# edogariu/artist-style-transfer

Hardware: NVIDIA B200
Metric: train_images_per_sec_256 (higher is better)
Workload: dtype bf16

## Files before the change

artist_style_transfer_b200/csrc/conv_hx.cu:

```cuda
#include "px_common.cuh"

namespace ast {

constexpr int HX_EPI_WARPS = 8;
constexpr int HX_WPROD_WARP = 2 + HX_EPI_WARPS;
constexpr int HX_THREADS = 32 * (HX_WPROD_WARP + 1);
constexpr int HX_MAX_PBUF = 4;
constexpr int HX_MAX_WBUF = 4;
constexpr int HX_TW = 8;

struct HxParams {
  int mi, mj, tiles_i, tiles_j, n_img, n_slices, R;
  int ntaps, kchunks, kc, cout, flags;
  int nblk, cb, sy, soy, sox, cstat;
  int oy[4], ox[4];
  int dy_min, dx_min, ph, pw;
  int patch_bytes, patch_tx, n_pbuf, n_wbuf, tg, ngroups;
  unsigned idesc;
  long long total_tiles;
  short tdy[AST_MAX_TAPS];
  short tdx[AST_MAX_TAPS];
};

__device__ __forceinline__ void hx_tile(const HxParams& p, long long tile, int& slice, int& tj, int& ti, int& img) {
  long long r = tile;
  slice = (int)(r % p.n_slices); r /= p.n_slices;
  tj = (int)(r % p.tiles_j); r /= p.tiles_j;
  ti = (int)(r % p.tiles_i);
  img = (int)(r / p.tiles_i);
}

template <int KIND>
__global__ void __launch_bounds__(HX_THREADS, 1)
conv_hx_kernel(const __grid_constant__ CUtensorMap tm_in, const __grid_constant__ CUtensorMap tm_w, const HxParams p,
               const float* __restrict__ bias, const Img32 add, const Img32 mask, const Img32 out,
               double* __restrict__ stats) {
  extern __shared__ unsigned char smem_raw[];
  __shared__ __align__(8) unsigned long long pfull[HX_MAX_PBUF], pempty[HX_MAX_PBUF], wfull[HX_MAX_WBUF], wempty[HX_MAX_WBUF];
  __shared__ __align__(8) unsigned long long tfull_bar[2], tempty_bar[2];
  __shared__ unsigned tmem_slot;
  __shared__ unsigned s_tapoff[AST_MAX_TAPS];

  unsigned char* smem_p = (unsigned char*)(((uintptr_t)smem_raw + 1023) & ~(uintptr_t)1023);
  unsigned char* smem_w = smem_p + (size_t)p.n_pbuf * p.patch_bytes;
  const int warp = threadIdx.x >> 5, lane = threadIdx.x & 31;
  constexpr int W_TILE = 128 * 128;
  const int w_slot = p.tg * W_TILE;

  if (threadIdx.x == 0) {
    asm volatile("prefetch.tensormap [%0];" ::"l"(&tm_in) : "memory");
    asm volatile("prefetch.tensormap [%0];" ::"l"(&tm_w) : "memory");
    for (int s = 0; s < p.n_pbuf; ++s) { mbar_init(&pfull[s], 1); mbar_init(&pempty[s], 1); }
    for (int s = 0; s < p.n_wbuf; ++s) { mbar_init(&wfull[s], 1); mbar_init(&wempty[s], 1); }
    for (int a = 0; a < 2; ++a) { mbar_init(&tfull_bar[a], 1); mbar_init(&tempty_bar[a], 32 * HX_EPI_WARPS); }
    asm volatile("fence.mbarrier_init.release.cluster;" ::: "memory");
    asm volatile("fence.proxy.async.shared::cta;" ::: "memory");
  }
  if (threadIdx.x >= 64 && threadIdx.x - 64 < p.ntaps) {
    const int t = threadIdx.x - 64;
    s_tapoff[t] = (unsigned)((p.tdy[t] * p.pw + p.tdx[t]) * 128) >> 4;
  }
  if (warp == 1) {
    asm volatile("tcgen05.alloc.cta_group::1.sync.aligned.shared::cta.b32 [%0], %1;" ::"r"(smem_u32(&tmem_slot)), "r"(512u) : "memory");
    asm volatile("tcgen05.relinquish_alloc_permit.cta_group::1.sync.aligned;" ::: "memory");
  }
  tc_fence_before();
  __syncthreads();
  tc_fence_after();
  const unsigned tmem_base = tmem_slot;

  if (warp == 0) {
    if (lane == 0) {
      int s = 0; unsigned ph = 0;
      for (long long tile = blockIdx.x; tile < p.total_tiles; tile += gridDim.x) {
        int slice, tj, ti, img;
        hx_tile(p, tile, slice, tj, ti, img);
        const int x0 = tj * HX_TW + p.dx_min, y0 = ti * p.R * p.sy + p.dy_min;
        for (int kc = 0; kc < p.kchunks; ++kc) {
          mbar_wait(&pempty[s], ph ^ 1);
          mbar_expect_tx(&pfull[s], (unsigned)p.patch_tx);
          tma_load_4d(smem_p + (size_t)s * p.patch_bytes, &tm_in, &pfull[s], kc * p.kc, x0, y0, img);
          if (++s == p.n_pbuf) { s = 0; ph ^= 1; }
        }
      }
    }
  } else if (warp == HX_WPROD_WARP) {
    if (lane == 0) {
      int s = 0; unsigned ph = 0;
      for (long long tile = blockIdx.x; tile < p.total_tiles; tile += gridDim.x) {
        int slice, tj, ti, img;
        hx_tile(p, tile, slice, tj, ti, img);
        for (int kc = 0; kc < p.kchunks; ++kc) {
          for (int gidx = 0; gidx < p.ngroups; ++gidx) {
            mbar_wait(&wempty[s], ph ^ 1);
            mbar_expect_tx(&wfull[s], (unsigned)w_slot);
            tma_load_3d(smem_w + (size_t)s * w_slot, &tm_w, &wfull[s], kc * p.kc, slice * 128, gidx * p.tg);
            if (++s == p.n_wbuf) { s = 0; ph ^= 1; }
          }
        }
      }
    }
  } else if (warp == 1) {
    int ps = 0; unsigned pph = 0; int ws = 0; unsigned wph = 0; int as = 0; unsigned aph = 0;
    const unsigned hi_w = ((8u * 128u) >> 4) | (1u << 14) | (2u << 29);
    const unsigned hi_p = (((unsigned)(p.sy * p.pw) * 128u) >> 4) | (1u << 14) | (2u << 29);
    const unsigned w_base = smem_u32(smem_w), p_base = smem_u32(smem_p);
    for (long long tile = blockIdx.x; tile < p.total_tiles; tile += gridDim.x) {
      mbar_wait(&tempty_bar[as], aph ^ 1);
      tc_fence_after();
      const unsigned d_tmem = tmem_base + (unsigned)(as * 256);
      for (int kc = 0; kc < p.kchunks; ++kc) {
        mbar_wait(&pfull[ps], pph);
        const unsigned p_lo = (((p_base + (unsigned)ps * (unsigned)p.patch_bytes) & 0x3FFFFu) >> 4) | (1u << 16);
        for (int gidx = 0; gidx < p.ngroups; ++gidx) {
          mbar_wait(&wfull[ws], wph);
          tc_fence_after();
          if (lane == 0) {
            const unsigned w_lo = (((w_base + (unsigned)ws * (unsigned)w_slot) & 0x3FFFFu) >> 4) | (1u << 16);
            const int t0 = gidx * p.tg, t1 = min(p.ntaps, t0 + p.tg);
            for (int t = t0; t < t1; ++t) {
              const unsigned a_lo = w_lo + (unsigned)(t - t0) * (W_TILE >> 4);
              const unsigned b_lo = p_lo + s_tapoff[t];
              tc_mma<KIND>(d_tmem, pack_desc64(a_lo, hi_w), pack_desc64(b_lo, hi_p), p.idesc, (kc | t) ? 1u : 0u);
              tc_mma<KIND>(d_tmem, pack_desc64(a_lo + 2, hi_w), pack_desc64(b_lo + 2, hi_p), p.idesc, 1u);
              tc_mma<KIND>(d_tmem, pack_desc64(a_lo + 4, hi_w), pack_desc64(b_lo + 4, hi_p), p.idesc, 1u);
              tc_mma<KIND>(d_tmem, pack_desc64(a_lo + 6, hi_w), pack_desc64(b_lo + 6, hi_p), p.idesc, 1u);
            }
            tc_commit(&wempty[ws]);
            if (gidx == p.ngroups - 1) {
              tc_commit(&pempty[ps]);
              if (kc == p.kchunks - 1) tc_commit(&tfull_bar[as]);
            }
          }
          __syncwarp();
          if (++ws == p.n_wbuf) { ws = 0; wph ^= 1; }
        }
        if (++ps == p.n_pbuf) { ps = 0; pph ^= 1; }
      }
      if (++as == 2) { as = 0; aph ^= 1; }
    }
  } else if (warp < HX_WPROD_WARP) {
    const int q = warp & 3;
    const int par = (warp - 2) >> 2;
    const int L = q * 32 + lane;
    const int blk = L / p.cb, chl = L % p.cb;
    const int oy_g = p.oy[blk], ox_g = p.ox[blk];
    PxStep st;
    st.out_r = p.soy * out.sh; st.out_c = p.sox * out.sw;
    st.add_r = p.soy * add.sh; st.add_c = p.sox * add.sw;
    st.mask_r = p.soy * mask.sh; st.mask_c = p.sox * mask.sw;
    const int jlim = min(p.mj, ox_g < out.w ? (out.w - ox_g + p.sox - 1) / p.sox : 0);
    const int ilim = min(p.mi, oy_g < out.h ? (out.h - oy_g + p.soy - 1) / p.soy : 0);
    int as = 0; unsigned aph = 0;
    double s1 = 0.0, s2 = 0.0;
    int s_img = -1, s_ch = 0;
    for (long long tile = blockIdx.x; tile < p.total_tiles; tile += gridDim.x) {
      int slice, tj, ti, img;
      hx_tile(p, tile, slice, tj, ti, img);
      const int ch = slice * 128 + chl;
      if (stats && (img != s_img || ch != s_ch)) {
        if (s_img >= 0) { double* srow = stats + ((long long)s_img * p.cstat + s_ch) * 2; atomicAdd(srow, s1); atomicAdd(srow + 1, s2); }
        s1 = s2 = 0.0; s_img = img; s_ch = ch;
      }
      const float b = bias ? bias[ch] : 0.f;
      mbar_wait(&tfull_bar[as], aph);
      tc_fence_after();
      const unsigned taddr0 = tmem_base + ((unsigned)(q * 32) << 16) + (unsigned)(as * 256);
      const int j0 = tj * HX_TW;
      const int nvc = max(0, min(HX_TW, jlim - j0));
#pragma unroll 1
      for (int c0 = par * 32; c0 < 256; c0 += 8 * HX_EPI_WARPS) {
        const int r0 = c0 >> 3;
        if (r0 >= p.R) break;
        float v[32];
        tc_ld32(taddr0 + c0, v);
        const int i0 = ti * p.R + r0;
        const int nvr = max(0, min(min(4, p.R - r0), ilim - i0));
        const int oy = oy_g + p.soy * i0, ox = ox_g + p.sox * j0;
        PxOff off;
        off.out = img * out.sn + oy * out.sh + ox * out.sw;
        off.add = add.ptr ? img * add.sn + oy * add.sh + ox * add.sw : 0;
        off.mask = mask.ptr ? img * mask.sn + oy * mask.sh + ox * mask.sw : 0;
        if (nvr == 4 && nvc == 8)
          px_chunk<8, true>(v, off, st, 4, 8, ch, lane, b, p.flags, add, mask, out, stats != nullptr, s1, s2);
        else if (nvr > 0 && nvc > 0)
          px_chunk<8>(v, off, st, nvr, nvc, ch, lane, b, p.flags, add, mask, out, stats != nullptr, s1, s2);
      }
      tc_fence_before();
      mbar_arrive(&tempty_bar[as]);
      if (++as == 2) { as = 0; aph ^= 1; }
    }
    if (stats && s_img >= 0) { double* srow = stats + ((long long)s_img * p.cstat + s_ch) * 2; atomicAdd(srow, s1); atomicAdd(srow + 1, s2); }
  }

  tc_fence_before();
  __syncthreads();
  if (warp == 1) {
    tc_fence_after();
    asm volatile("tcgen05.dealloc.cta_group::1.sync.aligned.b32 %0, %1;" ::"r"(tmem_base), "r"(512u) : "memory");
  }
}

struct HxGeom {
  int mi, mj, ntaps, flags;
  int nblk, cb, sy, soy, sox, cstat;
  int oy[4], ox[4];
  const int16_t* dy;
  const int16_t* dx;
  double* stats;
};

static int hx_launch(const ast_image* in, const void* weights, const float* bias, const ast_image* add, const ast_image* mask,
                     const ast_image* out, const HxGeom& g, int cout, cudaStream_t stream) {
  if (!img32_ok(out) || !img32_ok(add) || !img32_ok(mask)) return 0;
  const int esz = in->dtype == AST_F32 ? 4 : 2;
  if ((in->c * esz) % 128 != 0 || cout % 128 != 0) return 0;
  int dy_min = 1 << 30, dy_max = -(1 << 30), dx_min = 1 << 30, dx_max = -(1 << 30);
  for (int t = 0; t < g.ntaps; ++t) {
    dy_min = g.dy[t] < dy_min ? g.dy[t] : dy_min; dy_max = g.dy[t] > dy_max ? g.dy[t] : dy_max;
    dx_min = g.dx[t] < dx_min ? g.dx[t] : dx_min; dx_max = g.dx[t] > dx_max ? g.dx[t] : dx_max;
  }
  if (dx_max - dx_min > 4 || dy_max - dy_min > 8) return 0;
  HxParams p;
  memset(&p, 0, sizeof(p));
  p.kc = 128 / esz;
  p.kchunks = in->c / p.kc;
  if (g.ntaps * p.kchunks < 8) return 0;
  EncodeTiledFn encode = get_encode();
  if (!encode) return 0;
  p.mi = g.mi; p.mj = g.mj;
  p.nblk = g.nblk; p.cb = g.cb; p.sy = g.sy; p.soy = g.soy; p.sox = g.sox;
  for (int b = 0; b < 4; ++b) { p.oy[b] = g.oy[b]; p.ox[b] = g.ox[b]; }
  p.cstat = g.nblk == 1 ? cout : g.cb;
  p.ntaps = g.ntaps; p.flags = g.flags; p.cout = cout; p.n_img = in->n; p.n_slices = cout / 128;
  p.dy_min = dy_min; p.dx_min = dx_min;
  for (int t = 0; t < g.ntaps; ++t) { p.tdy[t] = g.dy[t] - dy_min; p.tdx[t] = g.dx[t] - dx_min; }
  p.pw = HX_TW + (dx_max - dx_min);
  const int budget = 225 * 1024 - 1024;
  p.tg = g.ntaps % 3 == 0 ? 3 : (g.ntaps % 2 == 0 ? 2 : (g.ntaps >= 3 ? 3 : g.ntaps));
  p.ngroups = (g.ntaps + p.tg - 1) / p.tg;
  const int w_slot = p.tg * 128 * 128;
  auto patch_rows = [&](int R) { return (R - 1) * p.sy + (dy_max - dy_min) + 1; };
  int rmax = 32;
  while (rmax > 2 && (2 * ((p.pw * patch_rows(rmax) * 128 + 1023) & ~1023) + 2 * w_slot > budget || patch_rows(rmax) > 256)) rmax -= 2;
  p.tiles_i = (p.mi + rmax - 1) / rmax;
  p.R = (p.mi + p.tiles_i - 1) / p.tiles_i;
  p.R = (p.R + 1) & ~1;
  p.tiles_i = (p.mi + p.R - 1) / p.R;
  p.tiles_j = (p.mj + HX_TW - 1) / HX_TW;
  p.total_tiles = (long long)p.n_img * p.tiles_i * p.tiles_j * p.n_slices;
  p.ph = patch_rows(p.R);
  p.patch_tx = p.pw * p.ph * 128;
  p.patch_bytes = (p.patch_tx + 1023) & ~1023;
  p.n_pbuf = 2;
  p.n_wbuf = (budget - p.n_pbuf * p.patch_bytes) / w_slot;
  if (p.n_wbuf < 2) return 0;
  if (p.n_wbuf > HX_MAX_WBUF) p.n_wbuf = HX_MAX_WBUF;
  if (budget - p.n_pbuf * p.patch_bytes - p.n_wbuf * w_slot >= p.patch_bytes) p.n_pbuf = 3;
  const unsigned fmt = tc_operand_fmt(in->dtype);
  p.idesc = (1u << 4) | (fmt << 7) | (fmt << 10) | ((unsigned)((8 * p.R) >> 3) << 17) | ((128u >> 4) << 24);

  alignas(64) CUtensorMap tm_in, tm_w;
  const CUtensorMapDataType dt = tc_tmap_dtype(in->dtype);
  {
    cuuint64_t dims[4] = {(cuuint64_t)in->c, (cuuint64_t)in->w, (cuuint64_t)in->h, (cuuint64_t)in->n};
    cuuint64_t strides[3] = {(cuuint64_t)in->sw * esz, (cuuint64_t)in->sh * esz, (cuuint64_t)in->sn * esz};
    cuuint32_t box[4] = {(cuuint32_t)p.kc, (cuuint32_t)p.pw, (cuuint32_t)p.ph, 1};
    cuuint32_t estr[4] = {1, 1, 1, 1};
    if (int r = cached_tensor_map(encode, &tm_in, dt, 4, in->ptr, dims, strides, box, estr, CU_TENSOR_MAP_SWIZZLE_128B,
                                  CU_TENSOR_MAP_L2_PROMOTION_L2_128B)) return r;
  }
  {
    cuuint64_t dims[3] = {(cuuint64_t)in->c, (cuuint64_t)cout, (cuuint64_t)g.ntaps};
    cuuint64_t strides[2] = {(cuuint64_t)in->c * esz, (cuuint64_t)cout * in->c * esz};
    cuuint32_t box[3] = {(cuuint32_t)p.kc, 128, (cuuint32_t)p.tg};
    cuuint32_t estr[3] = {1, 1, 1};
    if (int r = cached_tensor_map(encode, &tm_w, dt, 3, const_cast<void*>(weights), dims, strides, box, estr,
                                  CU_TENSOR_MAP_SWIZZLE_128B, CU_TENSOR_MAP_L2_PROMOTION_L2_256B)) return r;
  }
  const size_t smem = 1024 + (size_t)p.n_pbuf * p.patch_bytes + (size_t)p.n_wbuf * w_slot;
  const int grid = (int)(p.total_tiles < num_sms() ? p.total_tiles : num_sms());
  cudaError_t e;
  if (in->dtype != AST_F32) {
    e = set_max_smem(conv_hx_kernel<0>, smem);
    if (e == cudaSuccess) launch_k(conv_hx_kernel<0>, grid, HX_THREADS, smem, stream, tm_in, tm_w, p, bias, to_img32(add), to_img32(mask), to_img32(out), g.stats);
  } else {
    e = set_max_smem(conv_hx_kernel<1>, smem);
    if (e == cudaSuccess) launch_k(conv_hx_kernel<1>, grid, HX_THREADS, smem, stream, tm_in, tm_w, p, bias, to_img32(add), to_img32(mask), to_img32(out), g.stats);
  }
  if (e != cudaSuccess) { set_error("conv_hx: cudaFuncSetAttribute failed: %s", cudaGetErrorString(e)); return (int)e; }
  count_launch();
  return 1;
}

int conv_gather_hx(const ast_image* in, const void* weights, const float* bias, const ast_image* add,
                   const ast_image* mask, const ast_image* out, const ast_gather_geom* g, int cpad, bool thin,
                   cudaStream_t stream) {
  static const int enabled = [] { const char* e = getenv("AST_CONV_HX"); return e ? atoi(e) : 1; }();
  if (!enabled) return 0;
  if (thin || g->pooled || g->w_img_stride != 0 || g->si != 1 || cpad % 128 != 0 || out->c != cpad) return 0;
  int dy_min = 1 << 30, dy_max = -(1 << 30);
  for (int t = 0; t < g->ntaps; ++t) { dy_min = g->dy[t] < dy_min ? g->dy[t] : dy_min; dy_max = g->dy[t] > dy_max ? g->dy[t] : dy_max; }
  if (dy_max - dy_min > 4) return 0;
  HxGeom hg;
  memset(&hg, 0, sizeof(hg));
  hg.mi = g->mi; hg.mj = g->mj; hg.ntaps = g->ntaps; hg.flags = g->flags;
  hg.nblk = 1; hg.cb = 128; hg.sy = 1; hg.soy = hg.sox = g->so;
  hg.oy[0] = g->oy0; hg.ox[0] = g->ox0;
  hg.dy = g->dy; hg.dx = g->dx; hg.stats = g->stats;
  const int r = hx_launch(in, weights, bias, add, mask, out, hg, cpad, stream);
  if (r != 1) return r;
  count_work(FAM_CONV_HX, conv_flops(in, out, g), conv_bytes(in, out, g, add, mask));
  AST_CUDA_LAUNCH_CHECK();
  return 1;
}

int conv_stacked_hx(const ast_image* in, const void* weights, const float* bias, const ast_image* add,
                    const ast_image* mask, const ast_image* out, const ast_stacked_geom* g, cudaStream_t stream) {
  HxGeom hg;
  memset(&hg, 0, sizeof(hg));
  hg.mi = g->mi; hg.mj = g->mj; hg.ntaps = g->nvt; hg.flags = g->flags;
  hg.nblk = g->nblk; hg.cb = 128 / g->nblk; hg.sy = g->sy; hg.soy = g->soy; hg.sox = g->sox;
  for (int b = 0; b < g->nblk; ++b) { hg.oy[b] = g->oy[b]; hg.ox[b] = g->ox[b]; }
  hg.dy = g->dy; hg.dx = g->dx; hg.stats = g->stats;
  return hx_launch(in, weights, bias, add, mask, out, hg, 128, stream);
}

}
```

artist_style_transfer_b200/csrc/conv_px.cu:

```cuda
#include "px_common.cuh"

namespace ast {

constexpr int PX_THREADS = 320;
constexpr int PX_MAX_STAGES = 8;
constexpr int PX_PRODUCERS = 4;

struct PxParams {
  int mi, mj, tw, th, tiles_i, tiles_j, n_img;
  int ntaps, kchunks, kc;
  int si, so, oy0, ox0;
  int cout, flags;
  int w_rows_per_img;
  int stages, w_bytes, a_bytes, stage_bytes, rowb;
  int pairs_per_img;
  unsigned idesc, layout_type, sbo;
  long long total_pairs;
  short dy[AST_MAX_TAPS];
  short dx[AST_MAX_TAPS];
};

template <int KIND>
__global__ void __launch_bounds__(PX_THREADS, 1)
conv_px_kernel(const __grid_constant__ CUtensorMap tm_in, const __grid_constant__ CUtensorMap tm_w, const PxParams p,
               const float* __restrict__ bias, const Img32 add, const Img32 mask, const Img32 out,
               double* __restrict__ stats) {
  extern __shared__ unsigned char smem_raw[];
  __shared__ __align__(8) unsigned long long full_bar[PX_MAX_STAGES], empty_bar[PX_MAX_STAGES], tfull_bar[2], tempty_bar[2];
  __shared__ unsigned tmem_slot;
  unsigned char* smem = (unsigned char*)(((uintptr_t)smem_raw + 1023) & ~(uintptr_t)1023);
  const int warp = threadIdx.x >> 5, lane = threadIdx.x & 31;
  const int ksteps = p.ntaps * p.kchunks;

  if (threadIdx.x == 0) {
    asm volatile("prefetch.tensormap [%0];" ::"l"(&tm_in) : "memory");
    asm volatile("prefetch.tensormap [%0];" ::"l"(&tm_w) : "memory");
    for (int s = 0; s < p.stages; ++s) { mbar_init(&full_bar[s], 1); mbar_init(&empty_bar[s], 1); }
    for (int a = 0; a < 2; ++a) { mbar_init(&tfull_bar[a], 1); mbar_init(&tempty_bar[a], 256); }
    asm volatile("fence.mbarrier_init.release.cluster;" ::: "memory");
    asm volatile("fence.proxy.async.shared::cta;" ::: "memory");
  }
  if (warp == 1) {
    asm volatile("tcgen05.alloc.cta_group::1.sync.aligned.shared::cta.b32 [%0], %1;" ::"r"(smem_u32(&tmem_slot)), "r"(512u) : "memory");
    asm volatile("tcgen05.relinquish_alloc_permit.cta_group::1.sync.aligned;" ::: "memory");
  }
  tc_fence_before();
  __syncthreads();
  tc_fence_after();
  const unsigned tmem_base = tmem_slot;

  if (warp == 0) {
    const int nprod = p.stages < PX_PRODUCERS ? p.stages : PX_PRODUCERS;
    if (lane < nprod) {
      int s = 0, turn = 0; unsigned ph = 0;
      for (long long pair = blockIdx.x; pair < p.total_pairs; pair += gridDim.x) {
        const int img = (int)(pair / p.pairs_per_img);
        const int sp0 = 2 * (int)(pair % p.pairs_per_img);
        const int ti0 = sp0 / p.tiles_j, tj0 = sp0 - ti0 * p.tiles_j;
        const int ti1 = (sp0 + 1) / p.tiles_j, tj1 = (sp0 + 1) - ti1 * p.tiles_j;
        const int x0 = p.si * tj0 * p.tw, y0 = p.si * ti0 * p.th, x1 = p.si * tj1 * p.tw, y1 = p.si * ti1 * p.th;
        const int wrow0 = img * p.w_rows_per_img;
        for (int t = 0; t < p.ntaps; ++t) {
          for (int kc = 0; kc < p.kchunks; ++kc) {
            if (turn == lane) {
              mbar_wait(&empty_bar[s], ph ^ 1);
              unsigned char* sw = smem + (size_t)s * p.stage_bytes;
              mbar_expect_tx(&full_bar[s], (unsigned)p.stage_bytes);
              tma_load_2d(sw, &tm_w, &full_bar[s], kc * p.kc, wrow0 + t * p.cout);
              tma_load_4d(sw + p.w_bytes, &tm_in, &full_bar[s], kc * p.kc, x0 + p.dx[t], y0 + p.dy[t], img);
              tma_load_4d(sw + p.w_bytes + p.a_bytes, &tm_in, &full_bar[s], kc * p.kc, x1 + p.dx[t], y1 + p.dy[t], img);
            }
            if (++turn == nprod) turn = 0;
            if (++s == p.stages) { s = 0; ph ^= 1; }
          }
        }
      }
    }
  } else if (warp == 1) {
    int s = 0; unsigned ph = 0; int as = 0; unsigned aph = 0;
    const int kmma = p.rowb / 32;
    const unsigned desc_hi = (p.sbo >> 4) | (1u << 14) | (p.layout_type << 29);
    for (long long pair = blockIdx.x; pair < p.total_pairs; pair += gridDim.x) {
      mbar_wait(&tempty_bar[as], aph ^ 1);
      tc_fence_after();
      const unsigned d_tmem = tmem_base + (unsigned)(as * 256);
      for (int ks = 0; ks < ksteps; ++ks) {
        mbar_wait(&full_bar[s], ph);
        tc_fence_after();
        if (lane == 0) {
          const unsigned w_addr = smem_u32(smem + (size_t)s * p.stage_bytes);
          const unsigned a_lo = ((w_addr & 0x3FFFFu) >> 4) | (1u << 16);
          const unsigned b_lo = (((w_addr + p.w_bytes) & 0x3FFFFu) >> 4) | (1u << 16);
          tc_mma<KIND>(d_tmem, pack_desc64(a_lo, desc_hi), pack_desc64(b_lo, desc_hi), p.idesc, ks > 0 ? 1u : 0u);
          tc_mma<KIND>(d_tmem, pack_desc64(a_lo + 2, desc_hi), pack_desc64(b_lo + 2, desc_hi), p.idesc, 1u);
          if (kmma == 4) {
            tc_mma<KIND>(d_tmem, pack_desc64(a_lo + 4, desc_hi), pack_desc64(b_lo + 4, desc_hi), p.idesc, 1u);
            tc_mma<KIND>(d_tmem, pack_desc64(a_lo + 6, desc_hi), pack_desc64(b_lo + 6, desc_hi), p.idesc, 1u);
          }
          tc_commit(&empty_bar[s]);
          if (ks == ksteps - 1) tc_commit(&tfull_bar[as]);
        }
        __syncwarp();
        if (++s == p.stages) { s = 0; ph ^= 1; }
      }
      if (++as == 2) { as = 0; aph ^= 1; }
    }
  } else {
    const int q = warp & 3;
    const int half = (warp - 2) >> 2;
    const int ch = q * 32 + lane;
    const bool ch_ok = ch < p.cout;
    const float b = (bias && ch_ok) ? bias[ch] : 0.f;
    int as = 0; unsigned aph = 0;
    double s1 = 0.0, s2 = 0.0;
    int s_img = -1;
    for (long long pair = blockIdx.x; pair < p.total_pairs; pair += gridDim.x) {
      const int img = (int)(pair / p.pairs_per_img);
      if (stats && img != s_img) {
        if (s_img >= 0 && ch_ok) { double* srow = stats + ((long long)s_img * p.cout + ch) * 2; atomicAdd(srow, s1); atomicAdd(srow + 1, s2); }
        s1 = s2 = 0.0; s_img = img;
      }
      const int sp = 2 * (int)(pair % p.pairs_per_img) + half;
      const int ti = sp / p.tiles_j, tj = sp - ti * p.tiles_j;
      mbar_wait(&tfull_bar[as], aph);
      tc_fence_after();
      const unsigned taddr0 = tmem_base + ((unsigned)(q * 32) << 16) + (unsigned)(as * 256 + half * 128);
      if (q * 32 < p.cout) {
        const bool fast = (p.tw & 31) == 0;
        for (int c0 = 0; c0 < 128; c0 += 32) {
          float v[32];
          tc_ld32(taddr0 + c0, v);
          if (fast) {
            const int ty = c0 / p.tw, tx0 = c0 - ty * p.tw;
            const int i = ti * p.th + ty, j0 = tj * p.tw + tx0;
            const int oy = p.oy0 + p.so * i, ox = p.ox0 + p.so * j0;
            int nvalid = 0;
            if (i < p.mi && oy < out.h) {
              const int jlim = min(p.mj, (out.w - p.ox0 + p.so - 1) / p.so);
              nvalid = max(0, min(32, jlim - j0));
            }
            PxOff off;
            off.out = img * out.sn + oy * out.sh + ox * out.sw;
            off.add = add.ptr ? img * add.sn + oy * add.sh + ox * add.sw : 0;
            off.mask = mask.ptr ? img * mask.sn + oy * mask.sh + ox * mask.sw : 0;
            PxStep st;
            st.out_r = st.add_r = st.mask_r = 0;
            st.out_c = p.so * out.sw; st.add_c = p.so * add.sw; st.mask_c = p.so * mask.sw;
            if (nvalid > 0) px_chunk<32>(v, off, st, 1, nvalid, ch, lane, b, p.flags, add, mask, out, stats != nullptr, s1, s2);
          } else {
            const int row = c0 + lane;
            const int ty = row / p.tw, tx = row - ty * p.tw;
            const int i = ti * p.th + ty, j = tj * p.tw + tx;
            const int oy = p.oy0 + p.so * i, ox = p.ox0 + p.so * j;
            const bool valid = i < p.mi && j < p.mj && oy < out.h && ox < out.w;
            PxOff off;
            off.out = valid ? img * out.sn + oy * out.sh + ox * out.sw : -1;
            off.add = add.ptr ? img * add.sn + oy * add.sh + ox * add.sw : 0;
            off.mask = mask.ptr ? img * mask.sn + oy * mask.sh + ox * mask.sw : 0;
            PxStep st = {0, 0, 0, 0, 0, 0};
            px_chunk<0>(v, off, st, 0, 0, ch, lane, b, p.flags, add, mask, out, stats != nullptr, s1, s2);
          }
        }
      }
      tc_fence_before();
      mbar_arrive(&tempty_bar[as]);
      if (++as == 2) { as = 0; aph ^= 1; }
    }
    if (stats && s_img >= 0 && ch_ok) { double* srow = stats + ((long long)s_img * p.cout + ch) * 2; atomicAdd(srow, s1); atomicAdd(srow + 1, s2); }
  }

  tc_fence_before();
  __syncthreads();
  if (warp == 1) {
    tc_fence_after();
    asm volatile("tcgen05.dealloc.cta_group::1.sync.aligned.b32 %0, %1;" ::"r"(tmem_base), "r"(512u) : "memory");
  }
}

int conv_gather_px(const ast_image* in, const void* weights, const float* bias, const ast_image* add,
                   const ast_image* mask, const ast_image* out, const ast_gather_geom* g, int cpad, bool thin,
                   cudaStream_t stream) {
  if (thin || g->pooled || (cpad != 64 && cpad != 128) || out->c != cpad) return 0;
  if (!img32_ok(out) || !img32_ok(add) || !img32_ok(mask)) return 0;
  if (in->dtype == AST_F16) return 0;
  const int esz = in->dtype == AST_F32 ? 4 : 2;
  EncodeTiledFn encode = get_encode();
  if (!encode) return 0;

  PxParams p;
  memset(&p, 0, sizeof(p));
  p.mi = g->mi; p.mj = g->mj; p.si = g->si; p.so = g->so; p.oy0 = g->oy0; p.ox0 = g->ox0;
  p.ntaps = g->ntaps; p.flags = g->flags; p.cout = cpad; p.n_img = in->n;
  for (int t = 0; t < g->ntaps; ++t) { p.dy[t] = g->dy[t]; p.dx[t] = g->dx[t]; }
  pick_tile(p.mi, p.mj, 128, &p.tw, &p.th);
  p.tiles_i = (p.mi + p.th - 1) / p.th;
  p.tiles_j = (p.mj + p.tw - 1) / p.tw;
  p.rowb = (in->c * esz) % 128 == 0 ? 128 : 64;
  p.kc = p.rowb / esz;
  p.kchunks = in->c / p.kc;
  if (p.ntaps * p.kchunks * (p.rowb / 32) < 16) return 0;
  p.w_rows_per_img = 0;
  if (g->w_img_stride) {
    if (g->w_img_stride != (int64_t)g->ntaps * cpad * in->c) return 0;
    p.w_rows_per_img = g->ntaps * cpad;
  }
  p.w_bytes = 128 * p.rowb;
  p.a_bytes = 128 * p.rowb;
  p.stage_bytes = p.w_bytes + 2 * p.a_bytes;
  p.stages = (200 * 1024) / p.stage_bytes;
  if (p.stages > PX_MAX_STAGES) p.stages = PX_MAX_STAGES;
  p.layout_type = p.rowb == 128 ? 2u : 4u;
  p.sbo = 8u * p.rowb;
  const unsigned fmt = tc_operand_fmt(in->dtype);
  p.idesc = (1u << 4) | (fmt << 7) | (fmt << 10) | ((256u >> 3) << 17) | ((128u >> 4) << 24);
  p.pairs_per_img = (p.tiles_i * p.tiles_j + 1) / 2;
  p.total_pairs = (long long)p.n_img * p.pairs_per_img;

  alignas(64) CUtensorMap tm_in, tm_w;
  const CUtensorMapDataType dt = tc_tmap_dtype(in->dtype);
  const CUtensorMapSwizzle sw = p.rowb == 128 ? CU_TENSOR_MAP_SWIZZLE_128B : CU_TENSOR_MAP_SWIZZLE_64B;
  {
    cuuint64_t dims[4] = {(cuuint64_t)in->c, (cuuint64_t)in->w, (cuuint64_t)in->h, (cuuint64_t)in->n};
    cuuint64_t strides[3] = {(cuuint64_t)in->sw * esz, (cuuint64_t)in->sh * esz, (cuuint64_t)in->sn * esz};
    cuuint32_t box[4] = {(cuuint32_t)p.kc, (cuuint32_t)(p.tw * p.si), (cuuint32_t)(p.th * p.si), 1};
    cuuint32_t estr[4] = {1, (cuuint32_t)p.si, (cuuint32_t)p.si, 1};
    if (int r = cached_tensor_map(encode, &tm_in, dt, 4, in->ptr, dims, strides, box, estr, sw, CU_TENSOR_MAP_L2_PROMOTION_L2_128B)) return r;
  }
  {
    const long long rows = (long long)g->ntaps * cpad * (g->w_img_stride ? in->n : 1);
    cuuint64_t dims[2] = {(cuuint64_t)in->c, (cuuint64_t)rows};
    cuuint64_t strides[1] = {(cuuint64_t)in->c * esz};
    cuuint32_t box[2] = {(cuuint32_t)p.kc, 128};
    cuuint32_t estr[2] = {1, 1};
    if (int r = cached_tensor_map(encode, &tm_w, dt, 2, const_cast<void*>(weights), dims, strides, box, estr, sw, CU_TENSOR_MAP_L2_PROMOTION_L2_256B)) return r;
  }
  const size_t smem = (size_t)p.stages * p.stage_bytes + 1024;
  const int grid = (int)(p.total_pairs < num_sms() ? p.total_pairs : num_sms());
  cudaError_t e;
  if (in->dtype != AST_F32) {
    e = set_max_smem(conv_px_kernel<0>, smem);
    if (e == cudaSuccess) launch_k(conv_px_kernel<0>, grid, PX_THREADS, smem, stream, tm_in, tm_w, p, bias, to_img32(add), to_img32(mask), to_img32(out), g->stats);
  } else {
    e = set_max_smem(conv_px_kernel<1>, smem);
    if (e == cudaSuccess) launch_k(conv_px_kernel<1>, grid, PX_THREADS, smem, stream, tm_in, tm_w, p, bias, to_img32(add), to_img32(mask), to_img32(out), g->stats);
  }
  if (e != cudaSuccess) { set_error("conv_px: cudaFuncSetAttribute failed: %s", cudaGetErrorString(e)); return (int)e; }
  count_launch();
  count_work(FAM_CONV_PX, conv_flops(in, out, g), conv_bytes(in, out, g, add, mask));
  AST_CUDA_LAUNCH_CHECK();
  return 1;
}

}
```

artist_style_transfer_b200/csrc/conv_st.cu:

```cuda
#include "px_common.cuh"

namespace ast {

constexpr int ST_EPI_WARPS = 8;
constexpr int ST_THREADS = 64 + 32 * ST_EPI_WARPS;
constexpr int ST_MAX_PBUF = 4;
constexpr int ST_TW = 8;

struct StParams {
  int mi, mj, tiles_i, tiles_j, n_img, R;
  int nblk, cb, nvt, kchunks, kc, rowb, flags;
  int sy, soy, sox;
  int oy[4], ox[4];
  int dy_min, dx_min, ph, pw;
  int patch_bytes, patch_tx, n_pbuf, w_tile_bytes, w_total_bytes;
  unsigned idesc, layout_type;
  long long total_tiles;
  short tdy[AST_MAX_VTAPS];
  short tdx[AST_MAX_VTAPS];
};

__device__ __forceinline__ void st_tile(const StParams& p, long long tile, int& tj, int& ti, int& img) {
  long long r = tile;
  tj = (int)(r % p.tiles_j); r /= p.tiles_j;
  ti = (int)(r % p.tiles_i);
  img = (int)(r / p.tiles_i);
}

template <int KIND>
__global__ void __launch_bounds__(ST_THREADS, 1)
conv_st_kernel(const __grid_constant__ CUtensorMap tm_in, const __grid_constant__ CUtensorMap tm_w, const StParams p,
               const float* __restrict__ bias, const Img32 add, const Img32 mask, const Img32 out,
               double* __restrict__ stats) {
  extern __shared__ unsigned char smem_raw[];
  __shared__ __align__(8) unsigned long long pfull[ST_MAX_PBUF], pempty[ST_MAX_PBUF], tfull_bar[2], tempty_bar[2], wbar;
  __shared__ unsigned tmem_slot;
  __shared__ unsigned s_tapoff[AST_MAX_VTAPS];

  unsigned char* smem_w = (unsigned char*)(((uintptr_t)smem_raw + 1023) & ~(uintptr_t)1023);
  unsigned char* smem_p = smem_w + ((p.w_total_bytes + 1023) & ~1023);
  const int warp = threadIdx.x >> 5, lane = threadIdx.x & 31;

  if (threadIdx.x == 0) {
    asm volatile("prefetch.tensormap [%0];" ::"l"(&tm_in) : "memory");
    asm volatile("prefetch.tensormap [%0];" ::"l"(&tm_w) : "memory");
    for (int s = 0; s < p.n_pbuf; ++s) { mbar_init(&pfull[s], 1); mbar_init(&pempty[s], 1); }
    for (int a = 0; a < 2; ++a) { mbar_init(&tfull_bar[a], 1); mbar_init(&tempty_bar[a], 32 * ST_EPI_WARPS); }
    mbar_init(&wbar, 1);
    asm volatile("fence.mbarrier_init.release.cluster;" ::: "memory");
    asm volatile("fence.proxy.async.shared::cta;" ::: "memory");
  }
  if (threadIdx.x >= 64 && threadIdx.x - 64 < p.nvt) {
    const int t = threadIdx.x - 64;
    s_tapoff[t] = (unsigned)((p.tdy[t] * p.pw + p.tdx[t]) * p.rowb) >> 4;
  }
  if (warp == 1) {
    asm volatile("tcgen05.alloc.cta_group::1.sync.aligned.shared::cta.b32 [%0], %1;" ::"r"(smem_u32(&tmem_slot)), "r"(512u) : "memory");
    asm volatile("tcgen05.relinquish_alloc_permit.cta_group::1.sync.aligned;" ::: "memory");
  }
  tc_fence_before();
  __syncthreads();
  tc_fence_after();
  const unsigned tmem_base = tmem_slot;

  if (warp == 0) {
    if (lane == 0) {
      mbar_expect_tx(&wbar, (unsigned)p.w_total_bytes);
      for (int v = 0; v < p.nvt; ++v)
        for (int kc = 0; kc < p.kchunks; ++kc)
          tma_load_2d(smem_w + (size_t)(v * p.kchunks + kc) * p.w_tile_bytes, &tm_w, &wbar, kc * p.kc, v * 128);
      int s = 0; unsigned ph = 0;
      for (long long tile = tile_begin(p.total_tiles), tile_e = tile_end(p.total_tiles); tile < tile_e; ++tile) {
        int tj, ti, img;
        st_tile(p, tile, tj, ti, img);
        const int x0 = tj * ST_TW + p.dx_min, y0 = ti * p.R * p.sy + p.dy_min;
        for (int kc = 0; kc < p.kchunks; ++kc) {
          mbar_wait(&pempty[s], ph ^ 1);
          mbar_expect_tx(&pfull[s], (unsigned)p.patch_tx);
          tma_load_4d(smem_p + (size_t)s * p.patch_bytes, &tm_in, &pfull[s], kc * p.kc, x0, y0, img);
          if (++s == p.n_pbuf) { s = 0; ph ^= 1; }
        }
      }
    }
  } else if (warp == 1) {
    int s = 0; unsigned ph = 0; int as = 0; unsigned aph = 0;
    const int kmma = p.rowb / 32;
    mbar_wait(&wbar, 0);
    tc_fence_after();
    const unsigned hi_w = ((8u * (unsigned)p.rowb) >> 4) | (1u << 14) | (p.layout_type << 29);
    const unsigned hi_p = (((unsigned)(p.sy * p.pw * p.rowb)) >> 4) | (1u << 14) | (p.layout_type << 29);
    const unsigned w_lo0 = ((smem_u32(smem_w) & 0x3FFFFu) >> 4) | (1u << 16);
    const unsigned w16 = (unsigned)p.w_tile_bytes >> 4;
    for (long long tile = tile_begin(p.total_tiles), tile_e = tile_end(p.total_tiles); tile < tile_e; ++tile) {
      mbar_wait(&tempty_bar[as], aph ^ 1);
      tc_fence_after();
      const unsigned d_tmem = tmem_base + (unsigned)(as * 256);
      for (int kc = 0; kc < p.kchunks; ++kc) {
        mbar_wait(&pfull[s], ph);
        tc_fence_after();
        if (lane == 0) {
          const unsigned p_lo = ((smem_u32(smem_p + (size_t)s * p.patch_bytes) & 0x3FFFFu) >> 4) | (1u << 16);
          unsigned a_lo = w_lo0 + (unsigned)kc * w16;
          const unsigned a_step = (unsigned)p.kchunks * w16;
          unsigned acc = kc > 0 ? 1u : 0u;
#pragma unroll 2
          for (int v = 0; v < p.nvt; ++v) {
            const unsigned b_lo = p_lo + s_tapoff[v];
            tc_mma<KIND>(d_tmem, pack_desc64(a_lo, hi_w), pack_desc64(b_lo, hi_p), p.idesc, acc);
            tc_mma<KIND>(d_tmem, pack_desc64(a_lo + 2, hi_w), pack_desc64(b_lo + 2, hi_p), p.idesc, 1u);
            if (kmma == 4) {
              tc_mma<KIND>(d_tmem, pack_desc64(a_lo + 4, hi_w), pack_desc64(b_lo + 4, hi_p), p.idesc, 1u);
              tc_mma<KIND>(d_tmem, pack_desc64(a_lo + 6, hi_w), pack_desc64(b_lo + 6, hi_p), p.idesc, 1u);
            }
            acc = 1u;
            a_lo += a_step;
          }
          tc_commit(&pempty[s]);
          if (kc == p.kchunks - 1) tc_commit(&tfull_bar[as]);
        }
        __syncwarp();
        if (++s == p.n_pbuf) { s = 0; ph ^= 1; }
      }
      if (++as == 2) { as = 0; aph ^= 1; }
    }
  } else {
    const int q = warp & 3;
    const int par = (warp - 2) >> 2;
    const int L = q * 32 + lane;
    const int g = L / p.cb, ch = L % p.cb;
    const int oy_g = p.oy[g], ox_g = p.ox[g];
    PxStep st;
    st.out_r = p.soy * out.sh; st.out_c = p.sox * out.sw;
    st.add_r = p.soy * add.sh; st.add_c = p.sox * add.sw;
    st.mask_r = p.soy * mask.sh; st.mask_c = p.sox * mask.sw;
    const int ilim = min(p.mi, oy_g < out.h ? (out.h - oy_g + p.soy - 1) / p.soy : 0);
    const int jlim = min(p.mj, ox_g < out.w ? (out.w - ox_g + p.sox - 1) / p.sox : 0);
    const float b = bias ? bias[ch] : 0.f;
    int as = 0; unsigned aph = 0;
    double s1 = 0.0, s2 = 0.0;
    int s_img = -1;
    const int nchunks = (p.R + 3) >> 2;
    for (long long tile = tile_begin(p.total_tiles), tile_e = tile_end(p.total_tiles); tile < tile_e; ++tile) {
      int tj, ti, img;
      st_tile(p, tile, tj, ti, img);
      if (stats && img != s_img) {
        if (s_img >= 0) { double* srow = stats + ((long long)s_img * p.cb + ch) * 2; atomicAdd(srow, s1); atomicAdd(srow + 1, s2); }
        s1 = s2 = 0.0; s_img = img;
      }
      mbar_wait(&tfull_bar[as], aph);
      tc_fence_after();
      const unsigned taddr0 = tmem_base + ((unsigned)(q * 32) << 16) + (unsigned)(as * 256);
      const int j0 = tj * ST_TW;
      const int nvc = max(0, min(ST_TW, jlim - j0));
#pragma unroll 1
      for (int k = par; k < nchunks; k += ST_EPI_WARPS / 4) {
        float v[32];
        tc_ld32(taddr0 + (unsigned)(k * 32), v);
        const int r0 = k * 4;
        const int i0 = ti * p.R + r0;
        const int nvr = max(0, min(min(4, p.R - r0), ilim - i0));
        const int oy = oy_g + p.soy * i0, ox = ox_g + p.sox * j0;
        PxOff off;
        off.out = img * out.sn + oy * out.sh + ox * out.sw;
        off.add = add.ptr ? img * add.sn + oy * add.sh + ox * add.sw : 0;
        off.mask = mask.ptr ? img * mask.sn + oy * mask.sh + ox * mask.sw : 0;
        if (nvr == 4 && nvc == 8)
          px_chunk<8, true>(v, off, st, 4, 8, ch, lane, b, p.flags, add, mask, out, stats != nullptr, s1, s2);
        else if (nvr > 0 && nvc > 0)
          px_chunk<8>(v, off, st, nvr, nvc, ch, lane, b, p.flags, add, mask, out, stats != nullptr, s1, s2);
      }
      tc_fence_before();
      mbar_arrive(&tempty_bar[as]);
      if (++as == 2) { as = 0; aph ^= 1; }
    }
    if (stats && s_img >= 0) { double* srow = stats + ((long long)s_img * p.cb + ch) * 2; atomicAdd(srow, s1); atomicAdd(srow + 1, s2); }
  }

  tc_fence_before();
  __syncthreads();
  if (warp == 1) {
    tc_fence_after();
    asm volatile("tcgen05.dealloc.cta_group::1.sync.aligned.b32 %0, %1;" ::"r"(tmem_base), "r"(512u) : "memory");
  }
}

}

using namespace ast;

namespace ast {
int conv_stacked_hx(const ast_image* in, const void* weights, const float* bias, const ast_image* add,
                    const ast_image* mask, const ast_image* out, const ast_stacked_geom* g, cudaStream_t stream);
}

extern "C" int ast_conv_stacked(const ast_image* in, const void* weights, const float* bias, const ast_image* add,
                                const ast_image* mask, const ast_image* out, const ast_stacked_geom* g, void* stream) {
  AST_CHECK_ARG(in && weights && out && g, "ast_conv_stacked: null argument");
  AST_CHECK_ARG(g->nblk == 2 || g->nblk == 4, "ast_conv_stacked: nblk must be 2 or 4 (got %d)", g->nblk);
  AST_CHECK_ARG(g->nvt >= 1 && g->nvt <= AST_MAX_VTAPS, "ast_conv_stacked: nvt %d out of range", g->nvt);
  AST_CHECK_ARG(in->n == out->n, "ast_conv_stacked: batch mismatch %d vs %d", in->n, out->n);
  AST_CHECK_ARG(g->mi > 0 && g->mj > 0 && g->sy >= 1 && g->soy >= 1 && g->sox >= 1, "ast_conv_stacked: bad geometry");
  AST_CHECK_ARG(in->dtype == AST_F32 || in->dtype == AST_BF16 || in->dtype == AST_F16, "ast_conv_stacked: bad input dtype");
  AST_CHECK_ARG(out->dtype == AST_F32 || out->dtype == AST_BF16 || out->dtype == AST_F16, "ast_conv_stacked: bad output dtype");
  AST_CHECK_ARG(!add || same_shape(add, out), "ast_conv_stacked: add image shape mismatch");
  AST_CHECK_ARG(!mask || same_shape(mask, out), "ast_conv_stacked: mask image shape mismatch");
  const int cb = 128 / g->nblk;
  AST_CHECK_ARG(out->c == cb && out->sc == 1, "ast_conv_stacked: out must have %d contiguous channels (got %d)", cb, out->c);
  AST_CHECK_ARG(img32_ok(out) && img32_ok(add) && img32_ok(mask), "ast_conv_stacked: output images must span < 2^31 elements, sc = 1");
  AST_CHECK_ARG(in->sc == 1, "ast_conv_stacked: input must be channel-contiguous");
  if (in->n == 0) return 0;
  const int esz = in->dtype == AST_F32 ? 4 : 2;
  const int cbytes = in->c * esz;
  AST_CHECK_ARG(cbytes == 64 || cbytes % 128 == 0, "ast_conv_stacked: input pixels must be 64 bytes or a multiple of 128 bytes (got %d)", cbytes);
  int dy_min = 1 << 30, dy_max = -(1 << 30), dx_min = 1 << 30, dx_max = -(1 << 30);
  for (int t = 0; t < g->nvt; ++t) {
    dy_min = g->dy[t] < dy_min ? g->dy[t] : dy_min; dy_max = g->dy[t] > dy_max ? g->dy[t] : dy_max;
    dx_min = g->dx[t] < dx_min ? g->dx[t] : dx_min; dx_max = g->dx[t] > dx_max ? g->dx[t] : dx_max;
  }
  AST_CHECK_ARG(dx_max - dx_min <= 8, "ast_conv_stacked: horizontal tap span %d too wide", dx_max - dx_min);
  StParams p;
  memset(&p, 0, sizeof(p));
  p.rowb = cbytes == 64 ? 64 : 128;
  p.kc = p.rowb / esz;
  p.kchunks = in->c / p.kc;
  p.nblk = g->nblk; p.cb = cb; p.nvt = g->nvt; p.flags = g->flags;
  p.mi = g->mi; p.mj = g->mj; p.sy = g->sy; p.soy = g->soy; p.sox = g->sox; p.n_img = in->n;
  for (int b = 0; b < 4; ++b) { p.oy[b] = b < g->nblk ? g->oy[b] : 0; p.ox[b] = b < g->nblk ? g->ox[b] : 0; }
  p.dy_min = dy_min; p.dx_min = dx_min;
  for (int t = 0; t < g->nvt; ++t) { p.tdy[t] = g->dy[t] - dy_min; p.tdx[t] = g->dx[t] - dx_min; }
  p.w_tile_bytes = 128 * p.rowb;
  p.w_total_bytes = g->nvt * p.kchunks * p.w_tile_bytes;
  p.pw = ST_TW + (dx_max - dx_min);
  const int budget = 225 * 1024 - 1024 - ((p.w_total_bytes + 1023) & ~1023);
  auto patch_bytes = [&](int R) { return (p.pw * ((R - 1) * p.sy + (dy_max - dy_min) + 1) * p.rowb + 1023) & ~1023; };
  int rmax = 0;
  for (int nb = 3; nb >= 2 && !rmax; --nb)
    for (int R = 32; R >= (nb == 3 ? 16 : 2); R -= 2)
      if (nb * patch_bytes(R) <= budget && (R - 1) * p.sy + (dy_max - dy_min) + 1 <= 256) { rmax = R; break; }
  const double taps = (double)g->ntaps;
  const double pix = (double)in->n * g->mi * g->mj;
  const double flops = 2.0 * pix * taps * in->c * cb;
  double pix_in = (double)g->mi * g->sy * g->mj;
  if (pix_in > (double)in->h * in->w) pix_in = (double)in->h * in->w;
  const double bytes = in->n * pix_in * in->c * esize(in) +
                       pix * g->nblk * cb * (esize(out) + (add ? esize(add) : 0) + (mask ? esize(mask) : 0));
  if (rmax < 12) {
    const int r = conv_stacked_hx(in, weights, bias, add, mask, out, g, (cudaStream_t)stream);
    AST_CHECK_ARG(r != 0 || rmax > 0, "ast_conv_stacked: the stacked filter (%d bytes) neither fits in shared memory nor suits the streaming kernel", p.w_total_bytes);
    if (r == 1) {
      count_work(FAM_CONV_HX, flops, bytes);
      AST_CUDA_LAUNCH_CHECK();
      return 0;
    }
    if (r != 0) return r;
  }
  p.tiles_i = (p.mi + rmax - 1) / rmax;
  p.R = (p.mi + p.tiles_i - 1) / p.tiles_i;
  p.R = (p.R + 1) & ~1;
  p.tiles_i = (p.mi + p.R - 1) / p.R;
  p.tiles_j = (p.mj + ST_TW - 1) / ST_TW;
  p.total_tiles = (long long)p.n_img * p.tiles_i * p.tiles_j;
  p.ph = (p.R - 1) * p.sy + (dy_max - dy_min) + 1;
  p.patch_tx = p.pw * p.ph * p.rowb;
  p.patch_bytes = (p.patch_tx + 1023) & ~1023;
  p.n_pbuf = budget / p.patch_bytes;
  if (p.n_pbuf > ST_MAX_PBUF) p.n_pbuf = ST_MAX_PBUF;
  p.layout_type = p.rowb == 128 ? 2u : 4u;
  const unsigned fmt = tc_operand_fmt(in->dtype);
  p.idesc = (1u << 4) | (fmt << 7) | (fmt << 10) | ((unsigned)((8 * p.R) >> 3) << 17) | ((128u >> 4) << 24);

  EncodeTiledFn encode = get_encode();
  AST_CHECK_ARG(encode, "ast_conv_stacked: cuTensorMapEncodeTiled entry point not available");
  const CUtensorMapDataType dt = tc_tmap_dtype(in->dtype);
  const CUtensorMapSwizzle sw = p.rowb == 128 ? CU_TENSOR_MAP_SWIZZLE_128B : CU_TENSOR_MAP_SWIZZLE_64B;
  alignas(64) CUtensorMap tm_in, tm_w;
  {
    cuuint64_t dims[4] = {(cuuint64_t)in->c, (cuuint64_t)in->w, (cuuint64_t)in->h, (cuuint64_t)in->n};
    cuuint64_t strides[3] = {(cuuint64_t)in->sw * esz, (cuuint64_t)in->sh * esz, (cuuint64_t)in->sn * esz};
    cuuint32_t box[4] = {(cuuint32_t)p.kc, (cuuint32_t)p.pw, (cuuint32_t)p.ph, 1};
    cuuint32_t estr[4] = {1, 1, 1, 1};
    if (int r = cached_tensor_map(encode, &tm_in, dt, 4, in->ptr, dims, strides, box, estr, sw, CU_TENSOR_MAP_L2_PROMOTION_L2_128B)) return r;
  }
  {
    cuuint64_t dims[2] = {(cuuint64_t)in->c, (cuuint64_t)((long long)g->nvt * 128)};
    cuuint64_t strides[1] = {(cuuint64_t)in->c * esz};
    cuuint32_t box[2] = {(cuuint32_t)p.kc, 128};
    cuuint32_t estr[2] = {1, 1};
    if (int r = cached_tensor_map(encode, &tm_w, dt, 2, const_cast<void*>(weights), dims, strides, box, estr, sw, CU_TENSOR_MAP_L2_PROMOTION_L2_256B)) return r;
  }
  const size_t smem = 1024 + ((p.w_total_bytes + 1023) & ~1023) + (size_t)p.n_pbuf * p.patch_bytes;
  const int grid = (int)(p.total_tiles < num_sms() ? p.total_tiles : num_sms());
  cudaStream_t s = (cudaStream_t)stream;
  cudaError_t e;
  if (in->dtype != AST_F32) {
    e = set_max_smem(conv_st_kernel<0>, smem);
    if (e == cudaSuccess) launch_k(conv_st_kernel<0>, grid, ST_THREADS, smem, s, tm_in, tm_w, p, bias, to_img32(add), to_img32(mask), to_img32(out), g->stats);
  } else {
    e = set_max_smem(conv_st_kernel<1>, smem);
    if (e == cudaSuccess) launch_k(conv_st_kernel<1>, grid, ST_THREADS, smem, s, tm_in, tm_w, p, bias, to_img32(add), to_img32(mask), to_img32(out), g->stats);
  }
  if (e != cudaSuccess) { set_error("ast_conv_stacked: cudaFuncSetAttribute failed: %s", cudaGetErrorString(e)); return (int)e; }
  count_launch();
  count_work(FAM_CONV_ST, flops, bytes);
  AST_CUDA_LAUNCH_CHECK();
  return 0;
}
```

artist_style_transfer_b200/csrc/px_common.cuh:

```cuda
#pragma once
#include "tc_common.cuh"

namespace ast {

struct Img32 {
  char* ptr;
  int dtype, h, w, sn, sh, sw;
};

__device__ __forceinline__ float px_ld(const Img32& im, int off) {
  if (im.dtype == AST_F32) return reinterpret_cast<const float*>(im.ptr)[off];
  if (im.dtype == AST_F16) return __half2float(reinterpret_cast<const __half*>(im.ptr)[off]);
  return __bfloat162float(reinterpret_cast<const __nv_bfloat16*>(im.ptr)[off]);
}
__device__ __forceinline__ void px_st(const Img32& im, int off, float v) {
  if (im.dtype == AST_F32) reinterpret_cast<float*>(im.ptr)[off] = v;
  else if (im.dtype == AST_F16) reinterpret_cast<__half*>(im.ptr)[off] = f2h_sat(v);
  else reinterpret_cast<__nv_bfloat16*>(im.ptr)[off] = __float2bfloat16_rn(v);
}

struct PxOff { int out, add, mask; };
struct PxStep { int out_r, out_c, add_r, add_c, mask_r, mask_c; };
template <int CW, bool FULL = false>
__device__ __forceinline__ void px_chunk(float* v, const PxOff& off, const PxStep& st, int nvr, int nvc, int ch, int lane,
                                         float b, int flags, const Img32& add, const Img32& mask, const Img32& out,
                                         bool want_stats, double& s1, double& s2) {
  constexpr int W = CW ? CW : 1;
#define PX_OFF(f, idx) (CW ? off.f + ((idx) / W) * st.f##_r + ((idx) % W) * st.f##_c : __shfl_sync(0xffffffffu, off.f, (idx)))
#define PX_VALID(idx) (FULL ? true : (CW ? ((idx) / W < nvr && (idx) % W < nvc) : __shfl_sync(0xffffffffu, off.out, (idx)) >= 0))
#define PX_LOAD32_T(f, T, CVT, t)                                                                 \
  {                                                                                               \
    const T* base_ = reinterpret_cast<const T*>(f.ptr) + ch;                                      \
    _Pragma("unroll") for (int e = 0; e < 32; ++e) {                                              \
      const int o_ = PX_OFF(f, e);                                                                \
      t[e] = PX_VALID(e) ? CVT(base_[o_]) : 0.f;                                                  \
    }                                                                                             \
  }
#define PX_LOAD32(f, t)                                                                           \
  if (f.dtype == AST_F32) PX_LOAD32_T(f, float, float, t)                                         \
  else if (f.dtype == AST_F16) PX_LOAD32_T(f, __half, __half2float, t)                            \
  else PX_LOAD32_T(f, __nv_bfloat16, __bfloat162float, t)
  if (want_stats) {
    float sa[4] = {0.f, 0.f, 0.f, 0.f};
    int cnt = 0;
#pragma unroll
    for (int e = 0; e < 32; ++e)
      if (PX_VALID(e)) { sa[e & 3] += v[e]; ++cnt; }
    const float sum = (sa[0] + sa[1]) + (sa[2] + sa[3]);
    if (cnt > 0) {
      const float mu = sum / (float)cnt;
      float ma[4] = {0.f, 0.f, 0.f, 0.f};
#pragma unroll
      for (int e = 0; e < 32; ++e)
        if (PX_VALID(e)) { const float dlt = v[e] - mu; ma[e & 3] = fmaf(dlt, dlt, ma[e & 3]); }
      const float m2 = (ma[0] + ma[1]) + (ma[2] + ma[3]);
      s1 += (double)sum;
      s2 += (double)m2 + (double)cnt * ((double)mu * (double)mu);
    }
  }
  if (add.ptr) {
    float t[32];
    PX_LOAD32(add, t)
#pragma unroll
    for (int e = 0; e < 32; ++e) v[e] += t[e];
  }
  if (flags & AST_CONV_RELU) {
#pragma unroll
    for (int e = 0; e < 32; ++e) v[e] = fmaxf(v[e] + b, 0.f);
  } else if (b != 0.f) {
#pragma unroll
    for (int e = 0; e < 32; ++e) v[e] += b;
  }
  if (mask.ptr) {
    float t[32];
    PX_LOAD32(mask, t)
#pragma unroll
    for (int e = 0; e < 32; ++e) v[e] = t[e] > 0.f ? v[e] : 0.f;
  }
  if (flags & AST_CONV_ROUND_TF32) {
#pragma unroll
    for (int e = 0; e < 32; ++e) v[e] = round_tf32(v[e]);
  }
  if (out.dtype == AST_F32) {
#pragma unroll
    for (int e = 0; e < 32; ++e) {
      const int o = PX_OFF(out, e);
      if (FULL || (CW ? PX_VALID(e) : o >= 0)) reinterpret_cast<float*>(out.ptr)[o + ch] = v[e];
    }
  } else {
    const int odd = lane & 1;
    unsigned short* const obase = reinterpret_cast<unsigned short*>(out.ptr) + (ch & ~1);
    const int lane_off = CW ? off.out + odd * st.out_c : 0;
#define PX_STORE16(F16)                                                                           \
    _Pragma("unroll") for (int e = 0; e < 32; e += 2) {                                           \
      const float mine = odd ? v[e + 1] : v[e];                   \
      const float give = odd ? v[e] : v[e + 1];           \
      const float got = __shfl_xor_sync(0xffffffffu, give, 1);                                    \
      const int o = CW ? lane_off + (e / W) * st.out_r + (e % W) * st.out_c : PX_OFF(out, e + odd); \
      const bool ok = FULL || (CW ? PX_VALID(e + odd) : o >= 0);                                  \
      const unsigned pk = pack2<F16>(odd ? got : mine, odd ? mine : got);                         \
      if (ok) *reinterpret_cast<unsigned*>(obase + o) = pk;                                       \
    }
    if (out.dtype == AST_F16) { PX_STORE16(true) } else { PX_STORE16(false) }
#undef PX_STORE16
  }
#undef PX_LOAD32
#undef PX_LOAD32_T
#undef PX_VALID
#undef PX_OFF
}

inline bool img32_ok(const ast_image* im) {
  if (!im) return true;
  const long long span = (long long)(im->n - 1) * im->sn + (long long)(im->h - 1) * im->sh + (long long)(im->w - 1) * im->sw + im->c;
  return im->sc == 1 && im->sn >= 0 && im->sh >= 0 && im->sw >= 0 && span < (1ll << 31);
}
inline Img32 to_img32(const ast_image* im) {
  Img32 r;
  if (!im) { r.ptr = nullptr; r.dtype = 0; r.h = r.w = r.sn = r.sh = r.sw = 0; return r; }
  r.ptr = (char*)im->ptr; r.dtype = im->dtype; r.h = im->h; r.w = im->w;
  r.sn = (int)im->sn; r.sh = (int)im->sh; r.sw = (int)im->sw;
  return r;
}


}
```

artist_style_transfer_b200/csrc/tc_common.cuh:

```cuda
#pragma once
#include <cuda.h>

#include "common.cuh"

namespace ast {

__device__ __forceinline__ unsigned smem_u32(const void* p) { return (unsigned)__cvta_generic_to_shared(p); }

__device__ __forceinline__ void mbar_init(unsigned long long* bar, unsigned count) {
  asm volatile("mbarrier.init.shared::cta.b64 [%0], %1;" ::"r"(smem_u32(bar)), "r"(count));
}
__device__ __forceinline__ void mbar_expect_tx(unsigned long long* bar, unsigned bytes) {
  asm volatile("mbarrier.arrive.expect_tx.shared::cta.b64 _, [%0], %1;" ::"r"(smem_u32(bar)), "r"(bytes) : "memory");
}
__device__ __forceinline__ void mbar_arrive(unsigned long long* bar) {
  asm volatile("mbarrier.arrive.shared::cta.b64 _, [%0];" ::"r"(smem_u32(bar)) : "memory");
}
__device__ __forceinline__ void mbar_wait(unsigned long long* bar, unsigned parity) {
  const unsigned addr = smem_u32(bar);
  for (unsigned spin = 0; spin < (1u << 26); ++spin) {
    unsigned ok;
    asm volatile(
        "{\n"
        ".reg .pred p;\n"
        "mbarrier.try_wait.parity.shared::cta.b64 p, [%1], %2;\n"
        "selp.u32 %0, 1, 0, p;\n"
        "}\n"
        : "=r"(ok) : "r"(addr), "r"(parity) : "memory");
    if (ok) return;
  }
  __trap();
}
__device__ __forceinline__ void tma_load_4d(void* dst, const CUtensorMap* map, unsigned long long* bar, int c0, int c1,
                                            int c2, int c3) {
  asm volatile(
      "cp.async.bulk.tensor.4d.shared::cluster.global.mbarrier::complete_tx::bytes [%0], [%1, {%3, %4, %5, %6}], [%2];"
      ::"r"(smem_u32(dst)), "l"(map), "r"(smem_u32(bar)), "r"(c0), "r"(c1), "r"(c2), "r"(c3)
      : "memory");
}
__device__ __forceinline__ void tma_load_3d(void* dst, const CUtensorMap* map, unsigned long long* bar, int c0, int c1, int c2) {
  asm volatile(
      "cp.async.bulk.tensor.3d.shared::cluster.global.mbarrier::complete_tx::bytes [%0], [%1, {%3, %4, %5}], [%2];"
      ::"r"(smem_u32(dst)), "l"(map), "r"(smem_u32(bar)), "r"(c0), "r"(c1), "r"(c2)
      : "memory");
}
__device__ __forceinline__ void tma_load_2d(void* dst, const CUtensorMap* map, unsigned long long* bar, int c0, int c1) {
  asm volatile(
      "cp.async.bulk.tensor.2d.shared::cluster.global.mbarrier::complete_tx::bytes [%0], [%1, {%3, %4}], [%2];"
      ::"r"(smem_u32(dst)), "l"(map), "r"(smem_u32(bar)), "r"(c0), "r"(c1)
      : "memory");
}
__device__ __forceinline__ void tc_fence_before() { asm volatile("tcgen05.fence::before_thread_sync;" ::: "memory"); }
__device__ __forceinline__ void tc_fence_after() { asm volatile("tcgen05.fence::after_thread_sync;" ::: "memory"); }
__device__ __forceinline__ void tc_commit(unsigned long long* bar) {
  asm volatile("tcgen05.commit.cta_group::1.mbarrier::arrive::one.shared::cluster.b64 [%0];" ::"r"(smem_u32(bar))
               : "memory");
}
template <int KIND>
__device__ __forceinline__ void tc_mma(unsigned d_tmem, unsigned long long adesc, unsigned long long bdesc,
                                       unsigned idesc, unsigned accumulate) {
  if (KIND == 0)
    asm volatile("{\n.reg .pred p;\nsetp.ne.b32 p, %4, 0;\ntcgen05.mma.cta_group::1.kind::f16 [%0], %1, %2, %3, p;\n}\n"
                 ::"r"(d_tmem), "l"(adesc), "l"(bdesc), "r"(idesc), "r"(accumulate) : "memory");
  else
    asm volatile("{\n.reg .pred p;\nsetp.ne.b32 p, %4, 0;\ntcgen05.mma.cta_group::1.kind::tf32 [%0], %1, %2, %3, p;\n}\n"
                 ::"r"(d_tmem), "l"(adesc), "l"(bdesc), "r"(idesc), "r"(accumulate) : "memory");
}
__device__ __forceinline__ void tc_ld32(unsigned taddr, float* v) {
  unsigned r[32];
  asm volatile(
      "tcgen05.ld.sync.aligned.32x32b.x32.b32 "
      "{%0, %1, %2, %3, %4, %5, %6, %7, %8, %9, %10, %11, %12, %13, %14, %15, "
      "%16, %17, %18, %19, %20, %21, %22, %23, %24, %25, %26, %27, %28, %29, %30, %31}, [%32];"
      : "=r"(r[0]), "=r"(r[1]), "=r"(r[2]), "=r"(r[3]), "=r"(r[4]), "=r"(r[5]), "=r"(r[6]), "=r"(r[7]), "=r"(r[8]),
        "=r"(r[9]), "=r"(r[10]), "=r"(r[11]), "=r"(r[12]), "=r"(r[13]), "=r"(r[14]), "=r"(r[15]), "=r"(r[16]),
        "=r"(r[17]), "=r"(r[18]), "=r"(r[19]), "=r"(r[20]), "=r"(r[21]), "=r"(r[22]), "=r"(r[23]), "=r"(r[24]),
        "=r"(r[25]), "=r"(r[26]), "=r"(r[27]), "=r"(r[28]), "=r"(r[29]), "=r"(r[30]), "=r"(r[31])
      : "r"(taddr));
  asm volatile("tcgen05.wait::ld.sync.aligned;" ::: "memory");
#pragma unroll
  for (int i = 0; i < 32; ++i) v[i] = __uint_as_float(r[i]);
}
__device__ __forceinline__ unsigned long long make_smem_desc(unsigned saddr, unsigned sbo_bytes, unsigned layout_type) {
  unsigned long long d = 0;
  d |= (unsigned long long)((saddr & 0x3FFFFu) >> 4);
  d |= (unsigned long long)1 << 16;
  d |= (unsigned long long)(sbo_bytes >> 4) << 32;
  d |= (unsigned long long)1 << 46;
  d |= (unsigned long long)layout_type << 61;
  return d;
}
__device__ __forceinline__ unsigned long long pack_desc64(unsigned lo, unsigned hi) {
  unsigned long long d;
  asm("mov.b64 %0, {%1, %2};" : "=l"(d) : "r"(lo), "r"(hi));
  return d;
}
__device__ __forceinline__ float round_tf32(float x) {
  unsigned r;
  asm("cvt.rna.tf32.f32 %0, %1;" : "=r"(r) : "f"(x));
  return __uint_as_float(r);
}


#define LD4_EACH_T(im, off, T, BODY)                                                          \
  { _Pragma("unroll") for (int e = 0; e < 32; e += 4) { float t[4]; ld4((const T*)im.ptr + (off) + e, t); BODY } }
#define LD4_EACH(im, off, BODY)                                                               \
  if (im.dtype == AST_F32) LD4_EACH_T(im, off, float, BODY)                                   \
  else if (im.dtype == AST_F16) LD4_EACH_T(im, off, __half, BODY)                             \
  else LD4_EACH_T(im, off, __nv_bfloat16, BODY)
__device__ __forceinline__ void ld32_img(const Img& im, long long off, float* t) {
  if (im.dtype == AST_F32) {
#pragma unroll
    for (int e = 0; e < 32; e += 4) ld4((const float*)im.ptr + off + e, t + e);
  } else if (im.dtype == AST_F16) {
#pragma unroll
    for (int e = 0; e < 32; e += 8) {
      const uint4 u = *reinterpret_cast<const uint4*>((const __half*)im.ptr + off + e);
      const __half2* h = reinterpret_cast<const __half2*>(&u);
#pragma unroll
      for (int k = 0; k < 4; ++k) { const float2 f = __half22float2(h[k]); t[e + 2 * k] = f.x; t[e + 2 * k + 1] = f.y; }
    }
  } else {
#pragma unroll
    for (int e = 0; e < 32; e += 8) {
      const uint4 u = *reinterpret_cast<const uint4*>((const __nv_bfloat16*)im.ptr + off + e);
      const __nv_bfloat162* h = reinterpret_cast<const __nv_bfloat162*>(&u);
#pragma unroll
      for (int k = 0; k < 4; ++k) { const float2 f = __bfloat1622float2(h[k]); t[e + 2 * k] = f.x; t[e + 2 * k + 1] = f.y; }
    }
  }
}

__device__ __forceinline__ void tc_epilogue32(float* v, int co, int img, int oy, int ox, bool thin, int cout,
                                              int cout_valid, int flags, const float* __restrict__ bias, const Img& add,
                                              const Img& mask, const Img& out) {
  if (thin) {
#pragma unroll
    for (int e = 0; e < 32; ++e) {
      if (co + e >= cout_valid) continue;
      float x = v[e];
      if (bias) x += __ldg(bias + co + e);
      if (add.ptr) x += ld_elem(add, img_off(add, img, oy, ox, co + e));
      if (flags & AST_CONV_RELU) x = fmaxf(x, 0.f);
      if (mask.ptr) x = ld_elem(mask, img_off(mask, img, oy, ox, co + e)) > 0.f ? x : 0.f;
      if (flags & AST_CONV_ROUND_TF32) x = round_tf32(x);
      st_elem(out, img_off(out, img, oy, ox, co + e), x);
    }
    return;
  }
  if (co >= cout) return;
  if (bias) {
#pragma unroll
    for (int e = 0; e < 32; ++e) v[e] += __ldg(bias + co + e);
  }
  if (add.ptr) {
    const long long o = img_off(add, img, oy, ox, co);
    LD4_EACH(add, o, v[e] += t[0]; v[e + 1] += t[1]; v[e + 2] += t[2]; v[e + 3] += t[3];)
  }
  if (flags & AST_CONV_RELU) {
#pragma unroll
    for (int e = 0; e < 32; ++e) v[e] = fmaxf(v[e], 0.f);
  }
  if (mask.ptr) {
    const long long o = img_off(mask, img, oy, ox, co);
    LD4_EACH(mask, o, v[e] = t[0] > 0.f ? v[e] : 0.f; v[e + 1] = t[1] > 0.f ? v[e + 1] : 0.f; v[e + 2] = t[2] > 0.f ? v[e + 2] : 0.f; v[e + 3] = t[3] > 0.f ? v[e + 3] : 0.f;)
  }
  if (flags & AST_CONV_ROUND_TF32) {
#pragma unroll
    for (int e = 0; e < 32; ++e) v[e] = round_tf32(v[e]);
  }
  const long long oo = img_off(out, img, oy, ox, co);
  if (out.dtype == AST_F32) {
    float* op = (float*)out.ptr + oo;
#pragma unroll
    for (int e = 0; e < 32; e += 4) *reinterpret_cast<float4*>(op + e) = make_float4(v[e], v[e + 1], v[e + 2], v[e + 3]);
  } else {
    unsigned short* op = (unsigned short*)out.ptr + oo;
    if (out.dtype == AST_F16) {
#pragma unroll
      for (int e = 0; e < 32; e += 8)
        *reinterpret_cast<uint4*>(op + e) = make_uint4(pack2<true>(v[e], v[e + 1]), pack2<true>(v[e + 2], v[e + 3]),
                                                       pack2<true>(v[e + 4], v[e + 5]), pack2<true>(v[e + 6], v[e + 7]));
    } else {
#pragma unroll
      for (int e = 0; e < 32; e += 8)
        *reinterpret_cast<uint4*>(op + e) = make_uint4(pack2<false>(v[e], v[e + 1]), pack2<false>(v[e + 2], v[e + 3]),
                                                       pack2<false>(v[e + 4], v[e + 5]), pack2<false>(v[e + 6], v[e + 7]));
    }
  }
}

struct EpiRows { long long off[8]; };

__device__ __forceinline__ void tc_epi_stats_reduce(const float* v, bool valid, int lane, float& sum, float& sumsq) {
  float a[32], b[32];
#pragma unroll
  for (int e = 0; e < 32; ++e) { a[e] = valid ? v[e] : 0.f; b[e] = a[e] * a[e]; }
#pragma unroll
  for (int half = 16; half >= 1; half >>= 1) {
    const bool up = lane & half;
#pragma unroll
    for (int j = 0; j < half; ++j) {
      const float sa = up ? a[j] : a[j + half], ka = up ? a[j + half] : a[j];
      const float sb = up ? b[j] : b[j + half], kb = up ? b[j + half] : b[j];
      a[j] = ka + __shfl_xor_sync(0xffffffffu, sa, half);
      b[j] = kb + __shfl_xor_sync(0xffffffffu, sb, half);
    }
  }
  sum = a[0]; sumsq = b[0];
}
__device__ __forceinline__ long long tile_begin(long long total) { return total * (long long)blockIdx.x / (long long)gridDim.x; }
__device__ __forceinline__ long long tile_end(long long total) { return total * ((long long)blockIdx.x + 1) / (long long)gridDim.x; }

struct EpiStatAcc {
  double s[2][2];
  int img;
  __device__ __forceinline__ void reset(int image) { s[0][0] = s[0][1] = s[1][0] = s[1][1] = 0.0; img = image; }
  __device__ __forceinline__ void flush(double* __restrict__ stats, int cout, int co_first, int lane, int nchunks) {
    if (img < 0) return;
#pragma unroll
    for (int k = 0; k < 2; ++k) {
      if (k >= nchunks) break;
      double* row = stats + ((long long)img * cout + co_first + k * 64 + lane) * 2;
      atomicAdd(row, s[k][0]);
      atomicAdd(row + 1, s[k][1]);
    }
  }
};

__device__ __forceinline__ void sts128(unsigned addr, uint4 v) {
  asm volatile("st.shared.v4.b32 [%0], {%1, %2, %3, %4};" ::"r"(addr), "r"(v.x), "r"(v.y), "r"(v.z), "r"(v.w) : "memory");
}
__device__ __forceinline__ uint4 lds128(unsigned addr) {
  uint4 v;
  asm volatile("ld.shared.v4.b32 {%0, %1, %2, %3}, [%4];" : "=r"(v.x), "=r"(v.y), "=r"(v.z), "=r"(v.w) : "r"(addr) : "memory");
  return v;
}

__device__ __forceinline__ void tc_epi_row_offsets(long long my_off, int lane, bool f32, EpiRows& r) {
#pragma unroll
  for (int k = 0; k < 8; ++k) {
    const int src = f32 ? (8 * (k >> 1) + 4 * (k & 1) + (lane >> 3)) : (8 * (k & 3) + (lane >> 2));
    r.off[k] = __shfl_sync(0xffffffffu, my_off, src);
  }
}

__device__ __forceinline__ void tc_epi_prefetch_mask(const Img& mask, int img, int oy, int ox, int co, bool valid, float* m) {
  if (!mask.ptr || !valid) return;
  const long long o = img_off(mask, img, oy, ox, co);
  ld32_img(mask, o, m);
}

__device__ __forceinline__ void tc_epilogue32_coalesced(float* v, int co, int img, int oy, int ox, bool valid, int cout,
                                                        int flags, const float* __restrict__ bias, const Img& add,
                                                        const Img& mask, const Img& out, const EpiRows& rows,
                                                        unsigned char* stage, int lane, const float* pre_mask, bool have_pre) {
  if (co >= cout) return;
  if (valid) {
    if (bias) {
#pragma unroll
      for (int e = 0; e < 32; e += 4) {
        const float4 b4 = __ldg(reinterpret_cast<const float4*>(bias + co + e));
        v[e] += b4.x; v[e + 1] += b4.y; v[e + 2] += b4.z; v[e + 3] += b4.w;
      }
    }
    if (add.ptr) {
      const long long o = img_off(add, img, oy, ox, co);
      LD4_EACH(add, o, v[e] += t[0]; v[e + 1] += t[1]; v[e + 2] += t[2]; v[e + 3] += t[3];)
    }
    if (flags & AST_CONV_RELU) {
#pragma unroll
      for (int e = 0; e < 32; ++e) v[e] = fmaxf(v[e], 0.f);
    }
    if (mask.ptr && have_pre) {
#pragma unroll
      for (int e = 0; e < 32; ++e) v[e] = pre_mask[e] > 0.f ? v[e] : 0.f;
    } else if (mask.ptr) {
      const long long o = img_off(mask, img, oy, ox, co);
      LD4_EACH(mask, o, v[e] = t[0] > 0.f ? v[e] : 0.f; v[e + 1] = t[1] > 0.f ? v[e + 1] : 0.f; v[e + 2] = t[2] > 0.f ? v[e + 2] : 0.f; v[e + 3] = t[3] > 0.f ? v[e + 3] : 0.f;)
    }
    if (flags & AST_CONV_ROUND_TF32) {
#pragma unroll
      for (int e = 0; e < 32; ++e) v[e] = round_tf32(v[e]);
    }
  }
  const unsigned st = smem_u32(stage);
  const int r8 = lane & 7;
  if (out.dtype == AST_F32) {
    float* base = (float*)out.ptr + co + 4 * (lane & 7);
#pragma unroll
    for (int p = 0; p < 4; ++p) {
      if ((lane >> 3) == p) {
#pragma unroll
        for (int c = 0; c < 8; ++c)
          sts128(st + 16u * (r8 * 8 + (c ^ r8)), make_uint4(__float_as_uint(v[4 * c]), __float_as_uint(v[4 * c + 1]),
                                                             __float_as_uint(v[4 * c + 2]), __float_as_uint(v[4 * c + 3])));
      }
      __syncwarp();
#pragma unroll
      for (int i = 0; i < 2; ++i) {
        const int row = (lane >> 3) + 4 * i;
        const uint4 val = lds128(st + 16u * (row * 8 + ((lane & 7) ^ row)));
        const long long off = rows.off[2 * p + i];
        if (off >= 0) *reinterpret_cast<uint4*>(base + off) = val;
      }
      __syncwarp();
    }
  } else {
    unsigned short* base = (unsigned short*)out.ptr + co + 8 * (lane & 3);
    unsigned w[16];
    if (out.dtype == AST_F16) {
#pragma unroll
      for (int i = 0; i < 16; ++i) w[i] = pack2<true>(v[2 * i], v[2 * i + 1]);
    } else {
#pragma unroll
      for (int i = 0; i < 16; ++i) w[i] = pack2<false>(v[2 * i], v[2 * i + 1]);
    }
#pragma unroll
    for (int p = 0; p < 4; ++p) {
      if ((lane >> 3) == p) {
#pragma unroll
        for (int c = 0; c < 4; ++c)
          sts128(st + 16u * (r8 * 4 + (c ^ (r8 & 3))), make_uint4(w[4 * c], w[4 * c + 1], w[4 * c + 2], w[4 * c + 3]));
      }
      __syncwarp();
      {
        const int row = lane >> 2;
        const uint4 val = lds128(st + 16u * (row * 4 + ((lane & 3) ^ (row & 3))));
        const long long off = rows.off[p];
        if (off >= 0) *reinterpret_cast<uint4*>(base + off) = val;
      }
      __syncwarp();
    }
  }
}

typedef CUresult (*EncodeTiledFn)(CUtensorMap*, CUtensorMapDataType, cuuint32_t, void*, const cuuint64_t*,
                                  const cuuint64_t*, const cuuint32_t*, const cuuint32_t*, CUtensorMapInterleave,
                                  CUtensorMapSwizzle, CUtensorMapL2promotion, CUtensorMapFloatOOBfill);

inline EncodeTiledFn get_encode() {
  static EncodeTiledFn fn = nullptr;
  if (!fn) {
    void* p = nullptr;
    cudaDriverEntryPointQueryResult qres;
    if (cudaGetDriverEntryPoint("cuTensorMapEncodeTiled", &p, cudaEnableDefault, &qres) == cudaSuccess &&
        qres == cudaDriverEntryPointSuccess)
      fn = (EncodeTiledFn)p;
  }
  return fn;
}

int cached_tensor_map(EncodeTiledFn encode, CUtensorMap* out, CUtensorMapDataType dt, int rank, void* ptr,
                      const cuuint64_t* dims, const cuuint64_t* strides, const cuuint32_t* box, const cuuint32_t* estr,
                      CUtensorMapSwizzle sw, CUtensorMapL2promotion l2);
cudaError_t set_max_smem_impl(const void* kernel, size_t smem);
template <typename K> inline cudaError_t set_max_smem(K kernel, size_t smem) { return set_max_smem_impl((const void*)kernel, smem); }

inline CUtensorMapDataType tc_tmap_dtype(int dtype) {
  return dtype == AST_F32 ? CU_TENSOR_MAP_DATA_TYPE_FLOAT32 : (dtype == AST_F16 ? CU_TENSOR_MAP_DATA_TYPE_FLOAT16 : CU_TENSOR_MAP_DATA_TYPE_BFLOAT16);
}
inline unsigned tc_operand_fmt(int dtype) { return dtype == AST_F32 ? 2u : (dtype == AST_F16 ? 0u : 1u); }

inline void pick_tile(int mi, int mj, int area, int* tw, int* th) {
  double best = -1;
  for (int w = area; w >= 1; w >>= 1) {
    const int h = area / w;
    if (w > 256 || h > 256) continue;
    const double cover = (double)((mi + h - 1) / h * h) * ((mj + w - 1) / w * w);
    const double eff = (double)mi * mj / cover;
    if (eff > best + 1e-9) { best = eff; *tw = w; *th = h; }
  }
}

}
```

Baseline: 3483.

## Stage epilogue through per-warp shared memory and prefetch next TMEM chunk

Adds a staged epilogue path for the conv_px, conv_hx and conv_st tcgen05 kernels. Each epilogue warp gets its own shared-memory staging area, and the next TMEM chunk load is issued before the current chunk is stored, so TMEM reads overlap global stores. In conv_hx the staged variant is used only when residual add or mask inputs are present. Staging takes shared memory away from patch and weight buffers and pipeline stages, which can cut pipelining depth. conv_px's stage budget also changes from a fixed 200 KB to one derived from 225 KB minus the epilogue space.

```diff
diff --git a/artist_style_transfer_b200/csrc/conv_hx.cu b/artist_style_transfer_b200/csrc/conv_hx.cu
--- a/artist_style_transfer_b200/csrc/conv_hx.cu
+++ b/artist_style_transfer_b200/csrc/conv_hx.cu
@@ -16,6 +16,7 @@
   int oy[4], ox[4];
   int dy_min, dx_min, ph, pw;
   int patch_bytes, patch_tx, n_pbuf, n_wbuf, tg, ngroups;
+  int stage_warp_bytes;
   unsigned idesc;
   long long total_tiles;
   short tdy[AST_MAX_TAPS];
@@ -30,7 +31,7 @@
   img = (int)(r / p.tiles_i);
 }
 
-template <int KIND>
+template <int KIND, bool STAGED>
 __global__ void __launch_bounds__(HX_THREADS, 1)
 conv_hx_kernel(const __grid_constant__ CUtensorMap tm_in, const __grid_constant__ CUtensorMap tm_w, const HxParams p,
                const float* __restrict__ bias, const Img32 add, const Img32 mask, const Img32 out,
@@ -154,6 +155,7 @@
     int as = 0; unsigned aph = 0;
     double s1 = 0.0, s2 = 0.0;
     int s_img = -1, s_ch = 0;
+    const unsigned stage = smem_u32(smem_w + (size_t)p.n_wbuf * w_slot) + (unsigned)((warp - 2) * p.stage_warp_bytes);
     for (long long tile = blockIdx.x; tile < p.total_tiles; tile += gridDim.x) {
       int slice, tj, ti, img;
       hx_tile(p, tile, slice, tj, ti, img);
@@ -168,12 +170,15 @@
       const unsigned taddr0 = tmem_base + ((unsigned)(q * 32) << 16) + (unsigned)(as * 256);
       const int j0 = tj * HX_TW;
       const int nvc = max(0, min(HX_TW, jlim - j0));
+      float v[32];
+      if (STAGED && par * 4 < p.R) tc_ld32(taddr0 + par * 32, v);
 #pragma unroll 1
       for (int c0 = par * 32; c0 < 256; c0 += 8 * HX_EPI_WARPS) {
         const int r0 = c0 >> 3;
         if (r0 >= p.R) break;
-        float v[32];
-        tc_ld32(taddr0 + c0, v);
+        if (!STAGED) tc_ld32(taddr0 + c0, v);
+        const int cn = c0 + 8 * HX_EPI_WARPS;
+        const unsigned next = cn < 256 && (cn >> 3) < p.R ? taddr0 + cn : PX_NO_NEXT;
         const int i0 = ti * p.R + r0;
         const int nvr = max(0, min(min(4, p.R - r0), ilim - i0));
         const int oy = oy_g + p.soy * i0, ox = ox_g + p.sox * j0;
@@ -181,10 +186,19 @@
         off.out = img * out.sn + oy * out.sh + ox * out.sw;
         off.add = add.ptr ? img * add.sn + oy * add.sh + ox * add.sw : 0;
         off.mask = mask.ptr ? img * mask.sn + oy * mask.sh + ox * mask.sw : 0;
-        if (nvr == 4 && nvc == 8)
-          px_chunk<8, true>(v, off, st, 4, 8, ch, lane, b, p.flags, add, mask, out, stats != nullptr, s1, s2);
-        else if (nvr > 0 && nvc > 0)
-          px_chunk<8>(v, off, st, nvr, nvc, ch, lane, b, p.flags, add, mask, out, stats != nullptr, s1, s2);
+        if (STAGED) {
+          if (nvr == 4 && nvc == 8)
+            px_chunk_staged<8, true>(v, off, st, 4, 8, ch, lane, b, bias, p.flags, add, mask, out, stats != nullptr, s1, s2, stage, next);
+          else if (nvr > 0 && nvc > 0)
+            px_chunk_staged<8>(v, off, st, nvr, nvc, ch, lane, b, bias, p.flags, add, mask, out, stats != nullptr, s1, s2, stage, next);
+          else if (next != PX_NO_NEXT)
+            tc_ld32(next, v);
+        } else {
+          if (nvr == 4 && nvc == 8)
+            px_chunk<8, true>(v, off, st, 4, 8, ch, lane, b, p.flags, add, mask, out, stats != nullptr, s1, s2);
+          else if (nvr > 0 && nvc > 0)
+            px_chunk<8>(v, off, st, nvr, nvc, ch, lane, b, p.flags, add, mask, out, stats != nullptr, s1, s2);
+        }
       }
       tc_fence_before();
       mbar_arrive(&tempty_bar[as]);
@@ -236,7 +250,9 @@
   p.dy_min = dy_min; p.dx_min = dx_min;
   for (int t = 0; t < g.ntaps; ++t) { p.tdy[t] = g.dy[t] - dy_min; p.tdx[t] = g.dx[t] - dx_min; }
   p.pw = HX_TW + (dx_max - dx_min);
-  const int budget = 225 * 1024 - 1024;
+  p.stage_warp_bytes = add || mask ? px_stage_bytes(out, add, mask) : 0;
+  const int epi_bytes = HX_EPI_WARPS * p.stage_warp_bytes;
+  const int budget = 225 * 1024 - 1024 - epi_bytes;
   p.tg = g.ntaps % 3 == 0 ? 3 : (g.ntaps % 2 == 0 ? 2 : (g.ntaps >= 3 ? 3 : g.ntaps));
   p.ngroups = (g.ntaps + p.tg - 1) / p.tg;
   const int w_slot = p.tg * 128 * 128;
@@ -278,16 +294,13 @@
     if (int r = cached_tensor_map(encode, &tm_w, dt, 3, const_cast<void*>(weights), dims, strides, box, estr,
                                   CU_TENSOR_MAP_SWIZZLE_128B, CU_TENSOR_MAP_L2_PROMOTION_L2_256B)) return r;
   }
-  const size_t smem = 1024 + (size_t)p.n_pbuf * p.patch_bytes + (size_t)p.n_wbuf * w_slot;
+  const size_t smem = 1024 + (size_t)p.n_pbuf * p.patch_bytes + (size_t)p.n_wbuf * w_slot + epi_bytes;
   const int grid = (int)(p.total_tiles < num_sms() ? p.total_tiles : num_sms());
   cudaError_t e;
-  if (in->dtype != AST_F32) {
-    e = set_max_smem(conv_hx_kernel<0>, smem);
-    if (e == cudaSuccess) launch_k(conv_hx_kernel<0>, grid, HX_THREADS, smem, stream, tm_in, tm_w, p, bias, to_img32(add), to_img32(mask), to_img32(out), g.stats);
-  } else {
-    e = set_max_smem(conv_hx_kernel<1>, smem);
-    if (e == cudaSuccess) launch_k(conv_hx_kernel<1>, grid, HX_THREADS, smem, stream, tm_in, tm_w, p, bias, to_img32(add), to_img32(mask), to_img32(out), g.stats);
-  }
+  auto kernel = in->dtype != AST_F32 ? (epi_bytes ? conv_hx_kernel<0, true> : conv_hx_kernel<0, false>)
+                                     : (epi_bytes ? conv_hx_kernel<1, true> : conv_hx_kernel<1, false>);
+  e = set_max_smem(kernel, smem);
+  if (e == cudaSuccess) launch_k(kernel, grid, HX_THREADS, smem, stream, tm_in, tm_w, p, bias, to_img32(add), to_img32(mask), to_img32(out), g.stats);
   if (e != cudaSuccess) { set_error("conv_hx: cudaFuncSetAttribute failed: %s", cudaGetErrorString(e)); return (int)e; }
   count_launch();
   return 1;
diff --git a/artist_style_transfer_b200/csrc/conv_px.cu b/artist_style_transfer_b200/csrc/conv_px.cu
--- a/artist_style_transfer_b200/csrc/conv_px.cu
+++ b/artist_style_transfer_b200/csrc/conv_px.cu
@@ -14,13 +14,14 @@
   int w_rows_per_img;
   int stages, w_bytes, a_bytes, stage_bytes, rowb;
   int pairs_per_img;
+  int stage_warp_bytes;
   unsigned idesc, layout_type, sbo;
   long long total_pairs;
   short dy[AST_MAX_TAPS];
   short dx[AST_MAX_TAPS];
 };
 
-template <int KIND>
+template <int KIND, bool STAGED>
 __global__ void __launch_bounds__(PX_THREADS, 1)
 conv_px_kernel(const __grid_constant__ CUtensorMap tm_in, const __grid_constant__ CUtensorMap tm_w, const PxParams p,
                const float* __restrict__ bias, const Img32 add, const Img32 mask, const Img32 out,
@@ -114,6 +115,7 @@
     int as = 0; unsigned aph = 0;
     double s1 = 0.0, s2 = 0.0;
     int s_img = -1;
+    const unsigned stage = smem_u32(smem + (size_t)p.stages * p.stage_bytes) + (unsigned)((warp - 2) * p.stage_warp_bytes);
     for (long long pair = blockIdx.x; pair < p.total_pairs; pair += gridDim.x) {
       const int img = (int)(pair / p.pairs_per_img);
       if (stats && img != s_img) {
@@ -127,9 +129,11 @@
       const unsigned taddr0 = tmem_base + ((unsigned)(q * 32) << 16) + (unsigned)(as * 256 + half * 128);
       if (q * 32 < p.cout) {
         const bool fast = (p.tw & 31) == 0;
+        float v[32];
+        if (STAGED) tc_ld32(taddr0, v);
         for (int c0 = 0; c0 < 128; c0 += 32) {
-          float v[32];
-          tc_ld32(taddr0 + c0, v);
+          if (!STAGED) tc_ld32(taddr0 + c0, v);
+          const unsigned next = c0 + 32 < 128 ? taddr0 + c0 + 32 : PX_NO_NEXT;
           if (fast) {
             const int ty = c0 / p.tw, tx0 = c0 - ty * p.tw;
             const int i = ti * p.th + ty, j0 = tj * p.tw + tx0;
@@ -146,7 +150,12 @@
             PxStep st;
             st.out_r = st.add_r = st.mask_r = 0;
             st.out_c = p.so * out.sw; st.add_c = p.so * add.sw; st.mask_c = p.so * mask.sw;
-            if (nvalid > 0) px_chunk<32>(v, off, st, 1, nvalid, ch, lane, b, p.flags, add, mask, out, stats != nullptr, s1, s2);
+            if (nvalid > 0) {
+              if (STAGED) px_chunk_staged<32>(v, off, st, 1, nvalid, ch, lane, b, bias, p.flags, add, mask, out, stats != nullptr, s1, s2, stage, next);
+              else px_chunk<32>(v, off, st, 1, nvalid, ch, lane, b, p.flags, add, mask, out, stats != nullptr, s1, s2);
+            } else if (STAGED && next != PX_NO_NEXT) {
+              tc_ld32(next, v);
+            }
           } else {
             const int row = c0 + lane;
             const int ty = row / p.tw, tx = row - ty * p.tw;
@@ -158,7 +167,8 @@
             off.add = add.ptr ? img * add.sn + oy * add.sh + ox * add.sw : 0;
             off.mask = mask.ptr ? img * mask.sn + oy * mask.sh + ox * mask.sw : 0;
             PxStep st = {0, 0, 0, 0, 0, 0};
-            px_chunk<0>(v, off, st, 0, 0, ch, lane, b, p.flags, add, mask, out, stats != nullptr, s1, s2);
+            if (STAGED) px_chunk_staged<0>(v, off, st, 0, 0, ch, lane, b, bias, p.flags, add, mask, out, stats != nullptr, s1, s2, stage, next);
+            else px_chunk<0>(v, off, st, 0, 0, ch, lane, b, p.flags, add, mask, out, stats != nullptr, s1, s2);
           }
         }
       }
@@ -207,7 +217,9 @@
   p.w_bytes = 128 * p.rowb;
   p.a_bytes = 128 * p.rowb;
   p.stage_bytes = p.w_bytes + 2 * p.a_bytes;
-  p.stages = (200 * 1024) / p.stage_bytes;
+  p.stage_warp_bytes = px_stage_bytes(out, add, mask);
+  const int epi_bytes = 8 * p.stage_warp_bytes;
+  p.stages = (225 * 1024 - 1024 - epi_bytes) / p.stage_bytes;
   if (p.stages > PX_MAX_STAGES) p.stages = PX_MAX_STAGES;
   p.layout_type = p.rowb == 128 ? 2u : 4u;
   p.sbo = 8u * p.rowb;
@@ -234,16 +246,13 @@
     cuuint32_t estr[2] = {1, 1};
     if (int r = cached_tensor_map(encode, &tm_w, dt, 2, const_cast<void*>(weights), dims, strides, box, estr, sw, CU_TENSOR_MAP_L2_PROMOTION_L2_256B)) return r;
   }
-  const size_t smem = (size_t)p.stages * p.stage_bytes + 1024;
+  const size_t smem = (size_t)p.stages * p.stage_bytes + epi_bytes + 1024;
   const int grid = (int)(p.total_pairs < num_sms() ? p.total_pairs : num_sms());
   cudaError_t e;
-  if (in->dtype != AST_F32) {
-    e = set_max_smem(conv_px_kernel<0>, smem);
-    if (e == cudaSuccess) launch_k(conv_px_kernel<0>, grid, PX_THREADS, smem, stream, tm_in, tm_w, p, bias, to_img32(add), to_img32(mask), to_img32(out), g->stats);
-  } else {
-    e = set_max_smem(conv_px_kernel<1>, smem);
-    if (e == cudaSuccess) launch_k(conv_px_kernel<1>, grid, PX_THREADS, smem, stream, tm_in, tm_w, p, bias, to_img32(add), to_img32(mask), to_img32(out), g->stats);
-  }
+  auto kernel = in->dtype != AST_F32 ? (epi_bytes ? conv_px_kernel<0, true> : conv_px_kernel<0, false>)
+                                     : (epi_bytes ? conv_px_kernel<1, true> : conv_px_kernel<1, false>);
+  e = set_max_smem(kernel, smem);
+  if (e == cudaSuccess) launch_k(kernel, grid, PX_THREADS, smem, stream, tm_in, tm_w, p, bias, to_img32(add), to_img32(mask), to_img32(out), g->stats);
   if (e != cudaSuccess) { set_error("conv_px: cudaFuncSetAttribute failed: %s", cudaGetErrorString(e)); return (int)e; }
   count_launch();
   count_work(FAM_CONV_PX, conv_flops(in, out, g), conv_bytes(in, out, g, add, mask));
diff --git a/artist_style_transfer_b200/csrc/conv_st.cu b/artist_style_transfer_b200/csrc/conv_st.cu
--- a/artist_style_transfer_b200/csrc/conv_st.cu
+++ b/artist_style_transfer_b200/csrc/conv_st.cu
@@ -14,6 +14,7 @@
   int oy[4], ox[4];
   int dy_min, dx_min, ph, pw;
   int patch_bytes, patch_tx, n_pbuf, w_tile_bytes, w_total_bytes;
+  int stage_warp_bytes;
   unsigned idesc, layout_type;
   long long total_tiles;
   short tdy[AST_MAX_VTAPS];
@@ -27,7 +28,7 @@
   img = (int)(r / p.tiles_i);
 }
 
-template <int KIND>
+template <int KIND, bool STAGED>
 __global__ void __launch_bounds__(ST_THREADS, 1)
 conv_st_kernel(const __grid_constant__ CUtensorMap tm_in, const __grid_constant__ CUtensorMap tm_w, const StParams p,
                const float* __restrict__ bias, const Img32 add, const Img32 mask, const Img32 out,
@@ -140,6 +141,7 @@
     double s1 = 0.0, s2 = 0.0;
     int s_img = -1;
     const int nchunks = (p.R + 3) >> 2;
+    const unsigned stage = smem_u32(smem_p + (size_t)p.n_pbuf * p.patch_bytes) + (unsigned)((warp - 2) * p.stage_warp_bytes);
     for (long long tile = tile_begin(p.total_tiles), tile_e = tile_end(p.total_tiles); tile < tile_e; ++tile) {
       int tj, ti, img;
       st_tile(p, tile, tj, ti, img);
@@ -152,10 +154,13 @@
       const unsigned taddr0 = tmem_base + ((unsigned)(q * 32) << 16) + (unsigned)(as * 256);
       const int j0 = tj * ST_TW;
       const int nvc = max(0, min(ST_TW, jlim - j0));
+      float v[32];
+      if (STAGED && par < nchunks) tc_ld32(taddr0 + (unsigned)(par * 32), v);
 #pragma unroll 1
       for (int k = par; k < nchunks; k += ST_EPI_WARPS / 4) {
-        float v[32];
-        tc_ld32(taddr0 + (unsigned)(k * 32), v);
+        if (!STAGED) tc_ld32(taddr0 + (unsigned)(k * 32), v);
+        const int kn = k + ST_EPI_WARPS / 4;
+        const unsigned next = kn < nchunks ? taddr0 + (unsigned)(kn * 32) : PX_NO_NEXT;
         const int r0 = k * 4;
         const int i0 = ti * p.R + r0;
         const int nvr = max(0, min(min(4, p.R - r0), ilim - i0));
@@ -164,10 +169,19 @@
         off.out = img * out.sn + oy * out.sh + ox * out.sw;
         off.add = add.ptr ? img * add.sn + oy * add.sh + ox * add.sw : 0;
         off.mask = mask.ptr ? img * mask.sn + oy * mask.sh + ox * mask.sw : 0;
-        if (nvr == 4 && nvc == 8)
-          px_chunk<8, true>(v, off, st, 4, 8, ch, lane, b, p.flags, add, mask, out, stats != nullptr, s1, s2);
-        else if (nvr > 0 && nvc > 0)
-          px_chunk<8>(v, off, st, nvr, nvc, ch, lane, b, p.flags, add, mask, out, stats != nullptr, s1, s2);
+        if (STAGED) {
+          if (nvr == 4 && nvc == 8)
+            px_chunk_staged<8, true>(v, off, st, 4, 8, ch, lane, b, bias, p.flags, add, mask, out, stats != nullptr, s1, s2, stage, next);
+          else if (nvr > 0 && nvc > 0)
+            px_chunk_staged<8>(v, off, st, nvr, nvc, ch, lane, b, bias, p.flags, add, mask, out, stats != nullptr, s1, s2, stage, next);
+          else if (next != PX_NO_NEXT)
+            tc_ld32(next, v);
+        } else {
+          if (nvr == 4 && nvc == 8)
+            px_chunk<8, true>(v, off, st, 4, 8, ch, lane, b, p.flags, add, mask, out, stats != nullptr, s1, s2);
+          else if (nvr > 0 && nvc > 0)
+            px_chunk<8>(v, off, st, nvr, nvc, ch, lane, b, p.flags, add, mask, out, stats != nullptr, s1, s2);
+        }
       }
       tc_fence_before();
       mbar_arrive(&tempty_bar[as]);
@@ -231,7 +245,9 @@
   p.w_tile_bytes = 128 * p.rowb;
   p.w_total_bytes = g->nvt * p.kchunks * p.w_tile_bytes;
   p.pw = ST_TW + (dx_max - dx_min);
-  const int budget = 225 * 1024 - 1024 - ((p.w_total_bytes + 1023) & ~1023);
+  p.stage_warp_bytes = px_stage_bytes(out, add, mask);
+  const int epi_bytes = ST_EPI_WARPS * p.stage_warp_bytes;
+  const int budget = 225 * 1024 - 1024 - ((p.w_total_bytes + 1023) & ~1023) - epi_bytes;
   auto patch_bytes = [&](int R) { return (p.pw * ((R - 1) * p.sy + (dy_max - dy_min) + 1) * p.rowb + 1023) & ~1023; };
   int rmax = 0;
   for (int nb = 3; nb >= 2 && !rmax; --nb)
@@ -288,17 +304,14 @@
     cuuint32_t estr[2] = {1, 1};
     if (int r = cached_tensor_map(encode, &tm_w, dt, 2, const_cast<void*>(weights), dims, strides, box, estr, sw, CU_TENSOR_MAP_L2_PROMOTION_L2_256B)) return r;
   }
-  const size_t smem = 1024 + ((p.w_total_bytes + 1023) & ~1023) + (size_t)p.n_pbuf * p.patch_bytes;
+  const size_t smem = 1024 + ((p.w_total_bytes + 1023) & ~1023) + (size_t)p.n_pbuf * p.patch_bytes + epi_bytes;
   const int grid = (int)(p.total_tiles < num_sms() ? p.total_tiles : num_sms());
   cudaStream_t s = (cudaStream_t)stream;
   cudaError_t e;
-  if (in->dtype != AST_F32) {
-    e = set_max_smem(conv_st_kernel<0>, smem);
-    if (e == cudaSuccess) launch_k(conv_st_kernel<0>, grid, ST_THREADS, smem, s, tm_in, tm_w, p, bias, to_img32(add), to_img32(mask), to_img32(out), g->stats);
-  } else {
-    e = set_max_smem(conv_st_kernel<1>, smem);
-    if (e == cudaSuccess) launch_k(conv_st_kernel<1>, grid, ST_THREADS, smem, s, tm_in, tm_w, p, bias, to_img32(add), to_img32(mask), to_img32(out), g->stats);
-  }
+  auto kernel = in->dtype != AST_F32 ? (epi_bytes ? conv_st_kernel<0, true> : conv_st_kernel<0, false>)
+                                     : (epi_bytes ? conv_st_kernel<1, true> : conv_st_kernel<1, false>);
+  e = set_max_smem(kernel, smem);
+  if (e == cudaSuccess) launch_k(kernel, grid, ST_THREADS, smem, s, tm_in, tm_w, p, bias, to_img32(add), to_img32(mask), to_img32(out), g->stats);
   if (e != cudaSuccess) { set_error("ast_conv_stacked: cudaFuncSetAttribute failed: %s", cudaGetErrorString(e)); return (int)e; }
   count_launch();
   count_work(FAM_CONV_ST, flops, bytes);
diff --git a/artist_style_transfer_b200/csrc/px_common.cuh b/artist_style_transfer_b200/csrc/px_common.cuh
--- a/artist_style_transfer_b200/csrc/px_common.cuh
+++ b/artist_style_transfer_b200/csrc/px_common.cuh
@@ -21,6 +21,29 @@
 
 struct PxOff { int out, add, mask; };
 struct PxStep { int out_r, out_c, add_r, add_c, mask_r, mask_c; };
+template <int CW, bool FULL>
+__device__ __forceinline__ void px_stats(const float* v, const PxOff& off, int nvr, int nvc, double& s1, double& s2) {
+  constexpr int W = CW ? CW : 1;
+#define PX_VALID(idx) (FULL ? true : (CW ? ((idx) / W < nvr && (idx) % W < nvc) : __shfl_sync(0xffffffffu, off.out, (idx)) >= 0))
+  float sa[4] = {0.f, 0.f, 0.f, 0.f};
+  int cnt = 0;
+#pragma unroll
+  for (int e = 0; e < 32; ++e)
+    if (PX_VALID(e)) { sa[e & 3] += v[e]; ++cnt; }
+  const float sum = (sa[0] + sa[1]) + (sa[2] + sa[3]);
+  if (cnt > 0) {
+    const float mu = sum / (float)cnt;
+    float ma[4] = {0.f, 0.f, 0.f, 0.f};
+#pragma unroll
+    for (int e = 0; e < 32; ++e)
+      if (PX_VALID(e)) { const float dlt = v[e] - mu; ma[e & 3] = fmaf(dlt, dlt, ma[e & 3]); }
+    const float m2 = (ma[0] + ma[1]) + (ma[2] + ma[3]);
+    s1 += (double)sum;
+    s2 += (double)m2 + (double)cnt * ((double)mu * (double)mu);
+  }
+#undef PX_VALID
+}
+
 template <int CW, bool FULL = false>
 __device__ __forceinline__ void px_chunk(float* v, const PxOff& off, const PxStep& st, int nvr, int nvc, int ch, int lane,
                                          float b, int flags, const Img32& add, const Img32& mask, const Img32& out,
@@ -40,24 +63,7 @@
   if (f.dtype == AST_F32) PX_LOAD32_T(f, float, float, t)                                         \
   else if (f.dtype == AST_F16) PX_LOAD32_T(f, __half, __half2float, t)                            \
   else PX_LOAD32_T(f, __nv_bfloat16, __bfloat162float, t)
-  if (want_stats) {
-    float sa[4] = {0.f, 0.f, 0.f, 0.f};
-    int cnt = 0;
-#pragma unroll
-    for (int e = 0; e < 32; ++e)
-      if (PX_VALID(e)) { sa[e & 3] += v[e]; ++cnt; }
-    const float sum = (sa[0] + sa[1]) + (sa[2] + sa[3]);
-    if (cnt > 0) {
-      const float mu = sum / (float)cnt;
-      float ma[4] = {0.f, 0.f, 0.f, 0.f};
-#pragma unroll
-      for (int e = 0; e < 32; ++e)
-        if (PX_VALID(e)) { const float dlt = v[e] - mu; ma[e & 3] = fmaf(dlt, dlt, ma[e & 3]); }
-      const float m2 = (ma[0] + ma[1]) + (ma[2] + ma[3]);
-      s1 += (double)sum;
-      s2 += (double)m2 + (double)cnt * ((double)mu * (double)mu);
-    }
-  }
+  if (want_stats) px_stats<CW, FULL>(v, off, nvr, nvc, s1, s2);
   if (add.ptr) {
     float t[32];
     PX_LOAD32(add, t)
@@ -110,6 +116,192 @@
 #undef PX_OFF
 }
 
+constexpr int PX_STAGE_BYTES = 32 * 32 * 4;
+__device__ __forceinline__ unsigned px_word(const uint4& a, int k) { return k == 0 ? a.x : k == 1 ? a.y : k == 2 ? a.z : a.w; }
+constexpr unsigned PX_NO_NEXT = 0xffffffffu;
+
+template <int CW, bool FULL = false>
+__device__ __forceinline__ void px_chunk_staged(float* v, const PxOff& off, const PxStep& st, int nvr, int nvc, int ch,
+                                                int lane, float b, const float* __restrict__ bias, int flags,
+                                                const Img32& add, const Img32& mask, const Img32& out, bool want_stats,
+                                                double& s1, double& s2, unsigned stage, unsigned next_taddr) {
+  constexpr int W = CW ? CW : 1;
+  const int cg = lane & 3, pe = lane >> 2;
+  const int c0 = ch - lane + 8 * cg;
+  int oo[4], oa[4], om[4];
+  bool ok[4];
+#pragma unroll
+  for (int p = 0; p < 4; ++p) {
+    const int e = 8 * p + pe;
+    if (CW) {
+      const int r = e / W, c = e % W;
+      oo[p] = off.out + r * st.out_r + c * st.out_c + c0;
+      oa[p] = off.add + r * st.add_r + c * st.add_c + c0;
+      om[p] = off.mask + r * st.mask_r + c * st.mask_c + c0;
+      ok[p] = FULL || (r < nvr && c < nvc);
+    } else {
+      const int o = __shfl_sync(0xffffffffu, off.out, e);
+      oo[p] = o + c0;
+      oa[p] = add.ptr ? __shfl_sync(0xffffffffu, off.add, e) + c0 : 0;
+      om[p] = mask.ptr ? __shfl_sync(0xffffffffu, off.mask, e) + c0 : 0;
+      ok[p] = o >= 0;
+    }
+  }
+#define PX_LD_RAW(f, o, raw)                                                                      \
+  _Pragma("unroll") for (int p = 0; p < 4; ++p) {                                                 \
+    raw[p][0] = raw[p][1] = make_uint4(0u, 0u, 0u, 0u);                                           \
+    if (ok[p]) {                                                                                  \
+      const uint4* q_ = reinterpret_cast<const uint4*>(f.ptr + (size_t)o[p] * (f.dtype == AST_F32 ? 4 : 2)); \
+      raw[p][0] = q_[0];                                                                          \
+      if (f.dtype == AST_F32) raw[p][1] = q_[1];                                                  \
+    }                                                                                             \
+  }
+
+  if (want_stats) px_stats<CW, FULL>(v, off, nvr, nvc, s1, s2);
+  const bool wide = add.ptr != nullptr;
+  if (!add.ptr) {
+    if (flags & AST_CONV_RELU) {
+#pragma unroll
+      for (int e = 0; e < 32; ++e) v[e] = fmaxf(v[e] + b, 0.f);
+    } else if (b != 0.f) {
+#pragma unroll
+      for (int e = 0; e < 32; ++e) v[e] += b;
+    }
+    if (flags & AST_CONV_ROUND_TF32) {
+#pragma unroll
+      for (int e = 0; e < 32; ++e) v[e] = round_tf32(v[e]);
+    }
+  }
+  __syncwarp();
+  if (wide) {
+#pragma unroll
+    for (int e = 0; e < 32; ++e)
+      asm volatile("st.shared.b32 [%0], %1;" ::"r"(stage + 128u * e + 4u * (lane ^ ((e & 1) << 2))), "f"(v[e]) : "memory");
+  } else if (out.dtype == AST_F16) {
+#pragma unroll
+    for (int e = 0; e < 32; ++e)
+      asm volatile("st.shared.b16 [%0], %1;" ::"r"(stage + 64u * e + 2u * lane), "h"(__half_as_ushort(f2h_sat(v[e]))) : "memory");
+  } else {
+#pragma unroll
+    for (int e = 0; e < 32; ++e)
+      asm volatile("st.shared.b16 [%0], %1;" ::"r"(stage + 64u * e + 2u * lane), "h"(__bfloat16_as_ushort(__float2bfloat16_rn(v[e]))) : "memory");
+  }
+  if (next_taddr != PX_NO_NEXT) tc_ld32_issue(next_taddr, v);
+  __syncwarp();
+  uint4 mraw[4][2];
+  if (mask.ptr) PX_LD_RAW(mask, om, mraw)
+
+#define PX_CVT_RAW(f, raw, BODY)                                                                  \
+  if (f.dtype == AST_F32) {                                                                       \
+    _Pragma("unroll") for (int p = 0; p < 4; ++p) {                                               \
+      float t[8];                                                                                 \
+      _Pragma("unroll") for (int k = 0; k < 4; ++k) {                                             \
+        t[k] = __uint_as_float(px_word(raw[p][0], k)); t[4 + k] = __uint_as_float(px_word(raw[p][1], k)); \
+      }                                                                                           \
+      BODY                                                                                        \
+    }                                                                                             \
+  } else if (f.dtype == AST_F16) {                                                                \
+    _Pragma("unroll") for (int p = 0; p < 4; ++p) {                                               \
+      float t[8];                                                                                 \
+      _Pragma("unroll") for (int k = 0; k < 4; ++k) {                                             \
+        const unsigned w_ = px_word(raw[p][0], k);                                                \
+        const float2 f2_ = __half22float2(*reinterpret_cast<const __half2*>(&w_));               \
+        t[2 * k] = f2_.x; t[2 * k + 1] = f2_.y;                                                   \
+      }                                                                                           \
+      BODY                                                                                        \
+    }                                                                                             \
+  } else {                                                                                        \
+    _Pragma("unroll") for (int p = 0; p < 4; ++p) {                                               \
+      float t[8];                                                                                 \
+      _Pragma("unroll") for (int k = 0; k < 4; ++k) {                                             \
+        const unsigned w_ = px_word(raw[p][0], k);                                                \
+        const float2 f2_ = __bfloat1622float2(*reinterpret_cast<const __nv_bfloat162*>(&w_));     \
+        t[2 * k] = f2_.x; t[2 * k + 1] = f2_.y;                                                   \
+      }                                                                                           \
+      BODY                                                                                        \
+    }                                                                                             \
+  }
+  unsigned keep = 0xffffffffu;
+  if (mask.ptr) {
+    keep = 0;
+    PX_CVT_RAW(mask, mraw, _Pragma("unroll") for (int k = 0; k < 8; ++k) keep |= (t[k] > 0.f ? 1u : 0u) << (8 * p + k);)
+  }
+  if (wide) {
+    float x[4][8];
+#pragma unroll
+    for (int p = 0; p < 4; ++p) {
+      const int e = 8 * p + pe;
+#pragma unroll
+      for (int i = 0; i < 2; ++i) {
+        const uint4 u = lds128(stage + 128u * e + 16u * ((2 * cg + i) ^ (e & 1)));
+        x[p][4 * i] = __uint_as_float(u.x); x[p][4 * i + 1] = __uint_as_float(u.y);
+        x[p][4 * i + 2] = __uint_as_float(u.z); x[p][4 * i + 3] = __uint_as_float(u.w);
+      }
+    }
+    {
+      uint4 araw[4][2];
+      PX_LD_RAW(add, oa, araw)
+      PX_CVT_RAW(add, araw, _Pragma("unroll") for (int k = 0; k < 8; ++k) x[p][k] += t[k];)
+    }
+    float bb[8] = {0.f, 0.f, 0.f, 0.f, 0.f, 0.f, 0.f, 0.f};
+    if (bias) {
+      const float4 b0 = *reinterpret_cast<const float4*>(bias + c0), b1 = *reinterpret_cast<const float4*>(bias + c0 + 4);
+      bb[0] = b0.x; bb[1] = b0.y; bb[2] = b0.z; bb[3] = b0.w; bb[4] = b1.x; bb[5] = b1.y; bb[6] = b1.z; bb[7] = b1.w;
+    }
+#pragma unroll
+    for (int p = 0; p < 4; ++p)
+#pragma unroll
+      for (int k = 0; k < 8; ++k) {
+        if (flags & AST_CONV_RELU) x[p][k] = fmaxf(x[p][k] + bb[k], 0.f);
+        else if (bb[k] != 0.f) x[p][k] += bb[k];
+      }
+#pragma unroll
+    for (int p = 0; p < 4; ++p)
+#pragma unroll
+      for (int k = 0; k < 8; ++k) x[p][k] = (keep >> (8 * p + k)) & 1u ? x[p][k] : 0.f;
+    if (flags & AST_CONV_ROUND_TF32) {
+#pragma unroll
+      for (int p = 0; p < 4; ++p)
+#pragma unroll
+        for (int k = 0; k < 8; ++k) x[p][k] = round_tf32(x[p][k]);
+    }
+#define PX_STORE_PACKED(F16)                                                                      \
+    _Pragma("unroll") for (int p = 0; p < 4; ++p)                                                 \
+      if (ok[p])                                                                                  \
+        *reinterpret_cast<uint4*>(reinterpret_cast<unsigned short*>(out.ptr) + oo[p]) =           \
+            make_uint4(pack2<F16>(x[p][0], x[p][1]), pack2<F16>(x[p][2], x[p][3]),                \
+                       pack2<F16>(x[p][4], x[p][5]), pack2<F16>(x[p][6], x[p][7]));
+    if (out.dtype == AST_F16) { PX_STORE_PACKED(true) } else { PX_STORE_PACKED(false) }
+#undef PX_STORE_PACKED
+  } else {
+#pragma unroll
+    for (int p = 0; p < 4; ++p) {
+      const int e = 8 * p + pe;
+      uint4 u = lds128(stage + 64u * e + 16u * cg);
+      if (mask.ptr) {
+        const unsigned kb = keep >> (8 * p);
+#define PX_KEEP16(k) (((kb >> (2 * (k))) & 1u ? 0x0000ffffu : 0u) | ((kb >> (2 * (k) + 1)) & 1u ? 0xffff0000u : 0u))
+        u.x &= PX_KEEP16(0); u.y &= PX_KEEP16(1); u.z &= PX_KEEP16(2); u.w &= PX_KEEP16(3);
+#undef PX_KEEP16
+      }
+      if (ok[p]) *reinterpret_cast<uint4*>(reinterpret_cast<unsigned short*>(out.ptr) + oo[p]) = u;
+    }
+  }
+#undef PX_CVT_RAW
+#undef PX_LD_RAW
+  if (next_taddr != PX_NO_NEXT) tc_ld32_wait(v);
+}
+
+inline bool px_vec_ok(const ast_image* im) {
+  if (!im) return true;
+  const long long es = im->dtype == AST_F32 ? 4 : 2;
+  return ((uintptr_t)im->ptr & 15) == 0 && (im->sw * es) % 16 == 0 && (im->sh * es) % 16 == 0 && (im->sn * es) % 16 == 0;
+}
+inline int px_stage_bytes(const ast_image* out, const ast_image* add, const ast_image* mask) {
+  if (out->dtype == AST_F32 || !px_vec_ok(out) || !px_vec_ok(add) || !px_vec_ok(mask)) return 0;
+  return add ? PX_STAGE_BYTES : PX_STAGE_BYTES / 2;
+}
+
 inline bool img32_ok(const ast_image* im) {
   if (!im) return true;
   const long long span = (long long)(im->n - 1) * im->sn + (long long)(im->h - 1) * im->sh + (long long)(im->w - 1) * im->sw + im->c;
diff --git a/artist_style_transfer_b200/csrc/tc_common.cuh b/artist_style_transfer_b200/csrc/tc_common.cuh
--- a/artist_style_transfer_b200/csrc/tc_common.cuh
+++ b/artist_style_transfer_b200/csrc/tc_common.cuh
@@ -66,6 +66,22 @@
     asm volatile("{\n.reg .pred p;\nsetp.ne.b32 p, %4, 0;\ntcgen05.mma.cta_group::1.kind::tf32 [%0], %1, %2, %3, p;\n}\n"
                  ::"r"(d_tmem), "l"(adesc), "l"(bdesc), "r"(idesc), "r"(accumulate) : "memory");
 }
+__device__ __forceinline__ void tc_ld32_issue(unsigned taddr, float* v) {
+  asm volatile(
+      "tcgen05.ld.sync.aligned.32x32b.x32.b32 "
+      "{%0, %1, %2, %3, %4, %5, %6, %7, %8, %9, %10, %11, %12, %13, %14, %15, "
+      "%16, %17, %18, %19, %20, %21, %22, %23, %24, %25, %26, %27, %28, %29, %30, %31}, [%32];"
+      : "=f"(v[0]), "=f"(v[1]), "=f"(v[2]), "=f"(v[3]), "=f"(v[4]), "=f"(v[5]), "=f"(v[6]), "=f"(v[7]), "=f"(v[8]),
+        "=f"(v[9]), "=f"(v[10]), "=f"(v[11]), "=f"(v[12]), "=f"(v[13]), "=f"(v[14]), "=f"(v[15]), "=f"(v[16]),
+        "=f"(v[17]), "=f"(v[18]), "=f"(v[19]), "=f"(v[20]), "=f"(v[21]), "=f"(v[22]), "=f"(v[23]), "=f"(v[24]),
+        "=f"(v[25]), "=f"(v[26]), "=f"(v[27]), "=f"(v[28]), "=f"(v[29]), "=f"(v[30]), "=f"(v[31])
+      : "r"(taddr));
+}
+__device__ __forceinline__ void tc_ld32_wait(float* v) {
+  asm volatile("tcgen05.wait::ld.sync.aligned;" ::: "memory");
+#pragma unroll
+  for (int i = 0; i < 32; ++i) asm volatile("" : "+f"(v[i]));
+}
 __device__ __forceinline__ void tc_ld32(unsigned taddr, float* v) {
   unsigned r[32];
   asm volatile(
diff --git a/scratch/px_epilogue_ab.py b/scratch/px_epilogue_ab.py
--- /dev/null
+++ b/scratch/px_epilogue_ab.py
@@ -0,0 +1,170 @@
+import hashlib
+import os
+import pickle
+import sys
+
+import torch
+
+sys.path.insert(0, os.path.join(os.path.dirname(os.path.abspath(__file__)), ".."))
+
+TENSOR_ARGS = {"conv_gather": ("x", "wpacked", "out", "bias", "in_shift", "add", "mask", "stats", "pooled", "pool_codes"),
+               "conv_stacked": ("x", "wstacked", "out", "bias", "add", "mask", "stats")}
+
+
+def _meta(t):
+    st = t.untyped_storage()
+    return dict(key=st.data_ptr(), nbytes=st.nbytes(), dtype=t.dtype, offset=t.storage_offset(), shape=tuple(t.shape),
+                stride=tuple(t.stride()))
+
+
+def record(path, b, h, w):
+    import inspect
+    import artist_style_transfer_b200 as ast
+    from artist_style_transfer_b200 import ops
+    from oracle import weights
+    net = ast.StyleTransfer(device=torch.device("cuda"), precision="fast")
+    net.load_state_dict(weights.transfer_state_dict(2), strict=True)
+    vgg = ast.VGG16(vgg_path=None, precision="fast").cuda()
+    vgg.load_state_dict(weights.vgg_state_dict(2), strict=False)
+    content = weights.content_batch(b, h, 2, width=w).cuda()
+    style = ast.style_grams_single(vgg, weights.style_image(h, 2).cuda(), b)
+    calls = []
+    real = {n: getattr(ops, n) for n in TENSOR_ARGS}
+
+    def wrap(name):
+        def f(*args, **kwargs):
+            a = inspect.signature(real[name]).bind(*args, **kwargs)
+            a.apply_defaults()
+            rec = {"entry": name, "tensors": {}, "other": {}}
+            for k, v in a.arguments.items():
+                if isinstance(v, torch.Tensor):
+                    rec["tensors"][k] = _meta(v)
+                else:
+                    rec["other"][k] = v
+            calls.append(rec)
+            return real[name](*args, **kwargs)
+        return f
+    for n in TENSOR_ARGS:
+        setattr(ops, n, wrap(n))
+    ast.perceptual_step(net, vgg, content, style)
+    torch.cuda.synchronize()
+    for n in TENSOR_ARGS:
+        setattr(ops, n, real[n])
+    with open(path, "wb") as f:
+        pickle.dump(dict(workload=(b, h, w), calls=calls), f)
+    print(f"recorded {len(calls)} calls at B={b} {h}x{w}")
+
+
+def _make(rec, seed):
+    g = torch.Generator(device="cuda").manual_seed(seed)
+    stores = {}
+    args = {}
+    for role, m in rec["tensors"].items():
+        if m["key"] not in stores:
+            n = m["nbytes"] // torch.empty(0, dtype=m["dtype"]).element_size()
+            if m["dtype"] == torch.uint8:
+                s = torch.full((n,), 255, dtype=torch.uint8, device="cuda")
+            elif m["dtype"] == torch.float64:
+                s = torch.zeros(n, dtype=torch.float64, device="cuda")
+            else:
+                s = torch.randn(n, generator=g, device="cuda")
+                if role == "mask":
+                    s = s.clamp_min(0)
+                elif role in ("wpacked", "wstacked"):
+                    s = s * (1.0 / max(1, m["shape"][-1] * 9) ** 0.5)
+                elif role == "bias":
+                    s = s * 0.1
+                s = s.to(m["dtype"])
+            stores[m["key"]] = s
+        args[role] = torch.as_strided(stores[m["key"]], m["shape"], m["stride"], m["offset"])
+    return args, stores
+
+
+def _sha(t):
+    return hashlib.sha256(t.contiguous().view(torch.uint8).cpu().numpy().tobytes()).hexdigest()
+
+
+def run(calls_path, res_path, reps):
+    from artist_style_transfer_b200 import _lib, ops
+    with open(calls_path, "rb") as f:
+        d = pickle.load(f)
+    out = []
+    for i, rec in enumerate(d["calls"]):
+        args, stores = _make(rec, 1000 + i)
+        kw = dict(rec["other"])
+        kw.update(args)
+        fn = getattr(ops, rec["entry"])
+        fam0 = _lib.family_stats()
+        fn(**kw)
+        torch.cuda.synchronize()
+        fam = {k: v[0] for k, v in _lib.family_delta(fam0).items() if v[0]}
+        r = dict(entry=rec["entry"], fams=fam, out=tuple(args["out"].shape), out_dtype=str(args["out"].dtype)[6:],
+                 x=tuple(args["x"].shape), add="add" in args, mask="mask" in args, stats="stats" in args)
+        r["out_sha"] = _sha(stores[rec["tensors"]["out"]["key"]])
+        for k in ("pooled", "pool_codes"):
+            if k in args:
+                r[k + "_sha"] = _sha(stores[rec["tensors"][k]["key"]])
+        if "stats" in args:
+            r["stats_val"] = args["stats"].detach().cpu().clone()
+        if reps:
+            ts = []
+            for _ in range(reps):
+                e0, e1 = torch.cuda.Event(enable_timing=True), torch.cuda.Event(enable_timing=True)
+                e0.record()
+                fn(**kw)
+                e1.record()
+                e1.synchronize()
+                ts.append(e0.elapsed_time(e1) * 1e3)
+            ts.sort()
+            r["us"] = ts[len(ts) // 2]
+        out.append(r)
+        del args, stores, kw
+    torch.save(dict(workload=d["workload"], lib=os.environ.get("AST_B200_LIB", "in-tree"), calls=out), res_path)
+    print(f"ran {len(out)} calls with {os.environ.get('AST_B200_LIB', 'the in-tree library')}")
+
+
+def compare(a_path, b_path, *more):
+    A, B = torch.load(a_path), torch.load(b_path)
+    extra = [torch.load(p) for p in more]
+    bad = 0
+    fam_us = {}
+    print(f"workload B,H,W = {A['workload']}: A = {A['lib']}, B = {B['lib']}" + "".join(f", {e['lib']}" for e in extra))
+    for i, (a, b) in enumerate(zip(A["calls"], B["calls"])):
+        msgs = []
+        for k in ("out_sha", "pooled_sha", "pool_codes_sha"):
+            if a.get(k) != b.get(k):
+                msgs.append(f"{k} differs")
+        if a["fams"] != b["fams"]:
+            msgs.append(f"families {a['fams']} vs {b['fams']}")
+        if "stats_val" in a:
+            sa, sb = a["stats_val"], b["stats_val"]
+            rel = float(((sa - sb).abs() / sa.abs().clamp_min(1e-300)).max())
+            if not rel <= 1e-12:
+                msgs.append(f"stats rel {rel:.2e}")
+        bad += bool(msgs)
+        fam = "/".join(f"{k}x{v}" for k, v in a["fams"].items())
+        flags = ",".join(k for k in ("add", "mask", "stats") if a[k])
+        times = ""
+        if "us" in a:
+            times = f" {a['us']:8.1f} {b['us']:8.1f} us" + "".join(f" {e['calls'][i]['us']:8.1f}" for e in extra)
+            for f in a["fams"]:
+                t = fam_us.setdefault(f, [0.0, 0.0] + [0.0] * len(extra))
+                t[0] += a["us"]; t[1] += b["us"]
+                for j, e in enumerate(extra):
+                    t[2 + j] += e["calls"][i]["us"]
+        print(f"#{i:2d} {a['entry']:12s} {fam:18s} {str(a['x']):22s} -> {str(a['out']):22s} {a['out_dtype']:8s} "
+              f"[{flags}]{times} {'OK' if not msgs else 'MISMATCH: ' + '; '.join(msgs)}")
+    for f, t in sorted(fam_us.items()):
+        print(f"family {f}: " + " / ".join(f"{x / 1e3:.3f}" for x in t) + " ms (sum of per-call medians)")
+    print(f"{len(A['calls'])} calls, {bad} mismatching")
+    return bad
+
+
+if __name__ == "__main__":
+    cmd = sys.argv[1]
+    if cmd == "record":
+        record(sys.argv[2], int(sys.argv[3]), int(sys.argv[4]), int(sys.argv[5]))
+    elif cmd == "run":
+        run(sys.argv[2], sys.argv[3], int(sys.argv[4]) if len(sys.argv) > 4 else 0)
+    elif cmd == "compare":
+        sys.exit(1 if compare(*sys.argv[2:]) else 0)
```

Result: no change. 3504, median of 6 (+0.6%).
